# jgslunde/Lanczos

Measured on AMD Instinct MI355X. Metric: Lanczos iterations/sec + SpMV GB/s vs HBM roofline, n=1e7 5-pt Laplacian k=200, higher is better.
Workload: dtype f64

## Files before the change

### lanczos_amd/csrc/lz_api.hip

```cpp
#include <atomic>
#include <cstring>
#include <deque>
#include <unordered_map>

#include "lz_context.h"

using namespace lz;

namespace lz {
namespace api {

std::string g_create_error;


RcclApi g_rccl;

std::string g_rccl_path;
const char* load_rccl() {
  if (g_rccl.lib) return nullptr;
  void* lib = nullptr;
  std::vector<std::string> cand;
  if (const char* e = getenv("LZ_RCCL_PATH")) cand.push_back(e);
  Dl_info info;
  if (dladdr(reinterpret_cast<const void*>(static_cast<hipError_t (*)(void**, size_t)>(&hipMalloc)), &info) && info.dli_fname) {
    std::string dir(info.dli_fname);
    const size_t slash = dir.rfind('/');
    if (slash != std::string::npos) {
      dir.resize(slash);
      cand.push_back(dir + "/librccl.so.1");
      cand.push_back(dir + "/librccl.so");
    }
  }
  cand.push_back("/opt/rocm/lib/librccl.so.1");
  for (const auto& c : cand) {
    lib = dlopen(c.c_str(), RTLD_NOW | RTLD_LOCAL);
    if (lib) {
      g_rccl_path = c;
      break;
    }
  }
  if (!lib) return "cannot dlopen librccl next to the HIP runtime in use (set LZ_RCCL_PATH)";
#define LZ_SYM(field, name)                                          \
  g_rccl.field = reinterpret_cast<decltype(g_rccl.field)>(dlsym(lib, name)); \
  if (!g_rccl.field) return "missing RCCL symbol " name;
  LZ_SYM(GetUniqueId, "ncclGetUniqueId")
  LZ_SYM(CommInitRank, "ncclCommInitRank")
  LZ_SYM(CommDestroy, "ncclCommDestroy")
  LZ_SYM(AllReduce, "ncclAllReduce")
  LZ_SYM(AllGather, "ncclAllGather")
  LZ_SYM(Send, "ncclSend")
  LZ_SYM(Recv, "ncclRecv")
  LZ_SYM(GroupStart, "ncclGroupStart")
  LZ_SYM(GroupEnd, "ncclGroupEnd")
  LZ_SYM(GetErrorString, "ncclGetErrorString")
#undef LZ_SYM
  g_rccl.lib = lib;
  return nullptr;
}

int fail(lz_handle h, int code, const std::string& msg) {
  if (h)
    h->err = msg;
  else
    g_create_error = msg;
  return code;
}

int64_t skew_stride(lz_handle h, int64_t ld) {
  if (h->tune[12] == 1) return ld;
  return ((ld / kPadDoubles) & 1) ? ld : ld + kPadDoubles;
}

int check_launch(lz_handle h, const char* what) {
  hipError_t e = hipGetLastError();
  if (e != hipSuccess) return fail(h, LZ_ERR_HIP, std::string(what) + ": " + hipGetErrorString(e));
  if (h->tap_what && std::strcmp(what, h->tap_what) == 0)
    LZ_HIP(h, hipMemcpyAsync(h->d_tap, h->d_part, h->tap_count * sizeof(double), hipMemcpyDeviceToDevice, h->stream));
  return LZ_OK;
}

int upload(lz_handle h, void* dst, const void* src, size_t bytes) {
  LZ_HIP(h, hipMemcpyAsync(dst, src, bytes, hipMemcpyHostToDevice, h->stream));
  return LZ_OK;
}
int upload2d(lz_handle h, void* dst, size_t dpitch, const void* src, size_t spitch, size_t width, size_t height) {
  LZ_HIP(h, hipMemcpy2DAsync(dst, dpitch, src, spitch, width, height, hipMemcpyHostToDevice, h->stream));
  return LZ_OK;
}

namespace {
struct RoctxApi {
  int (*push)(const char*) = nullptr;
  int (*pop)() = nullptr;
  bool tried = false;
};
RoctxApi g_roctx;
const char* const kClassNames[LZ_K_COUNT] = {"lz:spmv", "lz:qtw", "lz:update", "lz:three_term", "lz:final", "lz:comm", "lz:ritz"};
bool roctx_on() {
  if (!g_roctx.tried) {
    g_roctx.tried = true;
    const char* e = getenv("LZ_ROCTX");
    if (e && e[0] == '1') {
      void* lib = dlopen("librocprofiler-sdk-roctx.so", RTLD_NOW | RTLD_GLOBAL);
      if (!lib) lib = dlopen("libroctx64.so", RTLD_NOW | RTLD_GLOBAL);
      if (lib) {
        g_roctx.push = reinterpret_cast<int (*)(const char*)>(dlsym(lib, "roctxRangePushA"));
        g_roctx.pop = reinterpret_cast<int (*)()>(dlsym(lib, "roctxRangePop"));
      }
    }
  }
  return g_roctx.push && g_roctx.pop;
}
}

Scope::Scope(lz_handle h_, int cls_, double bytes, double flops) : h(h_), cls(cls_) {
  if (roctx_on()) {
    g_roctx.push(kClassNames[cls]);
    marked = true;
  }
  h->acc.bytes[cls] += bytes;
  h->acc.flops[cls] += flops;
  h->acc.launches[cls] += 1;
  on = (h->flags & LZ_FLAG_PROFILE) != 0 && h->prof_iter;
  if (on) {
    h->acc.timed_bytes[cls] += bytes;
    h->acc.timed_launches[cls] += 1;
    if (!h->free_events.empty()) {
      a = h->free_events.back().first;
      b = h->free_events.back().second;
      h->free_events.pop_back();
    } else {
      if (hipEventCreate(&a) != hipSuccess || hipEventCreate(&b) != hipSuccess) {
        on = false;
        return;
      }
    }
    hipEventRecord(a, h->stream);
  }
}
Scope::~Scope() {
  if (marked) g_roctx.pop();
  if (on) {
    hipEventRecord(b, h->stream);
    h->events.push_back({cls, a, b});
  }
}

namespace {
struct BigBuf {
  size_t bytes = 0;
  std::vector<hipMemGenericAllocationHandle_t> chunks;
  std::vector<size_t> sizes;
};
std::mutex g_big_mu;
std::unordered_map<void*, BigBuf> g_big;
std::atomic<bool> g_vmm_off{false};
constexpr size_t kBigChunk = (size_t)2 << 30;
constexpr size_t kBigAlign = (size_t)2 << 20;

struct Quarantined {
  void* va;
  size_t bytes;
};
std::deque<Quarantined> g_quarantine;
size_t g_quarantine_bytes = 0;
constexpr size_t kQuarantineBytes = (size_t)16 << 40;

void big_release(void* va, BigBuf& b) {
  size_t off = 0;
  for (size_t k = 0; k < b.chunks.size(); ++k) {
    (void)hipMemUnmap(static_cast<char*>(va) + off, b.sizes[k]);
    (void)hipMemRelease(b.chunks[k]);
    off += b.sizes[k];
  }
  (void)hipMemAddressFree(va, b.bytes);
  static const bool reuse_ok = getenv("LZ_VMM_ADDRESS_REUSE") != nullptr;
  if (reuse_ok) return;
  void* q = nullptr;
  if (hipMemAddressReserve(&q, b.bytes, kBigAlign, va, 0) == hipSuccess && q) {
    if (q != va) {
      (void)hipMemAddressFree(q, b.bytes);
      if (getenv("LZ_DEBUG_VMM")) fprintf(stderr, "[vmm] quarantine of %p (%zu bytes) not honoured: got %p\n", va, b.bytes, q);
      return;
    }
    std::vector<Quarantined> old;
    {
      std::lock_guard<std::mutex> lk(g_big_mu);
      g_quarantine.push_back({q, b.bytes});
      g_quarantine_bytes += b.bytes;
      while (g_quarantine_bytes > kQuarantineBytes && g_quarantine.size() > 1) {
        old.push_back(g_quarantine.front());
        g_quarantine_bytes -= g_quarantine.front().bytes;
        g_quarantine.pop_front();
      }
    }
    for (const Quarantined& o : old) (void)hipMemAddressFree(o.va, o.bytes);
  } else {
    (void)hipGetLastError();
    if (getenv("LZ_DEBUG_VMM")) fprintf(stderr, "[vmm] quarantine of %p (%zu bytes): reservation failed\n", va, b.bytes);
  }
}
}

hipError_t big_alloc(int dev, void** out, size_t bytes) {
  *out = nullptr;
  static const bool no_vmm = getenv("LZ_NO_VMM") != nullptr;
  if (!no_vmm && !g_vmm_off.load() && bytes >= kBigMinBytes) {
    const size_t total = (bytes + kBigAlign - 1) / kBigAlign * kBigAlign;
    hipMemAllocationProp prop;
    memset(&prop, 0, sizeof prop);
    prop.type = hipMemAllocationTypePinned;
    prop.location.type = hipMemLocationTypeDevice;
    prop.location.id = dev;
    hipMemAccessDesc acc;
    acc.location.type = hipMemLocationTypeDevice;
    acc.location.id = dev;
    acc.flags = hipMemAccessFlagsProtReadWrite;
    void* va = nullptr;
    if (hipMemAddressReserve(&va, total, kBigAlign, nullptr, 0) == hipSuccess && va) {
      BigBuf b;
      b.bytes = total;
      bool ok = true, oom = false;
      for (size_t off = 0; off < total && ok; off += kBigChunk) {
        const size_t sz = std::min(kBigChunk, total - off);
        hipMemGenericAllocationHandle_t hh;
        hipError_t e = hipMemCreate(&hh, sz, &prop, 0);
        if (e != hipSuccess) {
          ok = false;
          oom = e == hipErrorOutOfMemory;
          break;
        }
        b.chunks.push_back(hh);
        b.sizes.push_back(sz);
        if (hipMemMap(static_cast<char*>(va) + off, sz, 0, hh, 0) != hipSuccess) {
          (void)hipMemRelease(hh);
          b.chunks.pop_back();
          b.sizes.pop_back();
          ok = false;
          break;
        }
        if (hipMemSetAccess(static_cast<char*>(va) + off, sz, &acc, 1) != hipSuccess) ok = false;
      }
      if (ok) {
        std::lock_guard<std::mutex> lk(g_big_mu);
        g_big.emplace(va, std::move(b));
        *out = va;
        return hipSuccess;
      }
      big_release(va, b);
      (void)hipGetLastError();
      if (oom) return hipErrorOutOfMemory;
    } else {
      (void)hipGetLastError();
    }
  }
  return hipMalloc(out, bytes);
}

void big_vmm_disable() { g_vmm_off.store(true); }

hipError_t big_free(void* p) {
  if (!p) return hipSuccess;
  BigBuf b;
  {
    std::lock_guard<std::mutex> lk(g_big_mu);
    auto it = g_big.find(p);
    if (it == g_big.end()) return hipFree(p);
    b = std::move(it->second);
    g_big.erase(it);
  }
  hipError_t e = hipDeviceSynchronize();
  big_release(p, b);
  return e;
}

int drain_events(lz_handle h) {
  if (h->events.empty() && !h->run_timed) return LZ_OK;
  LZ_HIP(h, hipStreamSynchronize(h->stream));
  for (auto& e : h->events) {
    float ms = 0.f;
    LZ_HIP(h, hipEventElapsedTime(&ms, e.a, e.b));
    h->acc.ms[e.cls] += ms;
    h->free_events.push_back({e.a, e.b});
  }
  h->events.clear();
  if (h->run_timed) {
    float ms = 0.f;
    LZ_HIP(h, hipEventElapsedTime(&ms, h->run_a, h->run_b));
    h->acc.total_ms += ms;
    h->run_timed = false;
  }
  return LZ_OK;
}

int comm_allreduce(lz_handle h, double* dbuf, int64_t count) {
  if ((h->world <= 1 && !(h->tune[6] && h->comm_kind)) || count <= 0) return LZ_OK;
  Scope sc(h, LZ_K_COMM, 8.0 * count, 0);
  h->n_allreduce += 1;
  if (h->comm_kind == 1) {
    LZ_NCCL(h, g_rccl.AllReduce(dbuf, dbuf, (size_t)count, ncclDouble, ncclSum, h->comm, h->stream));
    return LZ_OK;
  }
  if (h->comm_kind == 2) {
    h->hbuf_a.resize((size_t)count);
    LZ_HIP(h, hipMemcpyAsync(h->hbuf_a.data(), dbuf, count * sizeof(double), hipMemcpyDeviceToHost, h->stream));
    LZ_HIP(h, hipStreamSynchronize(h->stream));
    h->host_syncs += 2;
    if (h->h_ar(h->h_user, h->hbuf_a.data(), count) != 0) return fail(h, LZ_ERR_COMM, "host all-reduce callback failed");
    LZ_HIP(h, hipMemcpyAsync(dbuf, h->hbuf_a.data(), count * sizeof(double), hipMemcpyHostToDevice, h->stream));
    LZ_HIP(h, hipStreamSynchronize(h->stream));
    return LZ_OK;
  }
  return fail(h, LZ_ERR_STATE, "world > 1 but no communicator initialised");
}

int comm_exchange_x(lz_handle h, int j, const double** x_out) {
  double* vj = h->d_V + (int64_t)j * h->ldv;
  *x_out = vj;
  if (h->world <= 1 && !(h->tune[6] && h->comm_kind)) return LZ_OK;
  if (h->xmode == 1) {
    if (h->peers.empty()) return LZ_OK;
    Scope sc(h, LZ_K_COMM, 8.0 * (h->total_send + h->total_recv), 0);
    h->n_exchange += 1;
    const bool direct = h->all_contig && h->comm_kind == 1;
    if (!direct) {
      launch_gather(vj, h->d_send_idx, h->total_send, h->d_sendbuf, h->stream);
      LZ_TRY(check_launch(h, "gather"));
    }
    double* ghost = vj + h->rows_pad;
    if (h->comm_kind == 1) {
      LZ_NCCL(h, g_rccl.GroupStart());
      for (size_t p = 0; p < h->peers.size(); ++p) {
        const double* src = direct ? vj + h->sstart[p] : h->d_sendbuf + h->soff[p];
        if (h->scount[p] > 0)
          LZ_NCCL(h, g_rccl.Send(src, (size_t)h->scount[p], ncclDouble, h->peers[p], h->comm, h->stream));
        if (h->rcount[p] > 0)
          LZ_NCCL(h, g_rccl.Recv(ghost + h->roff[p], (size_t)h->rcount[p], ncclDouble, h->peers[p], h->comm, h->stream));
      }
      LZ_NCCL(h, g_rccl.GroupEnd());
    } else {
      h->hbuf_a.resize((size_t)std::max<int64_t>(h->total_send, 1));
      h->hbuf_b.resize((size_t)std::max<int64_t>(h->total_recv, 1));
      LZ_HIP(h, hipMemcpyAsync(h->hbuf_a.data(), h->d_sendbuf, h->total_send * sizeof(double), hipMemcpyDeviceToHost, h->stream));
      LZ_HIP(h, hipStreamSynchronize(h->stream));
      h->host_syncs += 2;
      if (h->h_ex(h->h_user, (int)h->peers.size(), h->peers.data(), h->hbuf_a.data(), h->scount.data(), h->hbuf_b.data(),
                  h->rcount.data()) != 0)
        return fail(h, LZ_ERR_COMM, "host halo-exchange callback failed");
      LZ_HIP(h, hipMemcpyAsync(ghost, h->hbuf_b.data(), h->total_recv * sizeof(double), hipMemcpyHostToDevice, h->stream));
      LZ_HIP(h, hipStreamSynchronize(h->stream));
    }
    return LZ_OK;
  }
  if (h->xmode == 2) {
    Scope sc(h, LZ_K_COMM, 8.0 * h->ag_chunk * h->world, 0);
    h->n_exchange += 1;
    if (h->comm_kind == 1) {
      LZ_NCCL(h, g_rccl.AllGather(vj, h->d_xfull, (size_t)h->ag_chunk, ncclDouble, h->comm, h->stream));
    } else {
      h->hbuf_a.resize((size_t)h->ag_chunk);
      h->hbuf_b.resize((size_t)(h->ag_chunk * h->world));
      LZ_HIP(h, hipMemcpyAsync(h->hbuf_a.data(), vj, h->ag_chunk * sizeof(double), hipMemcpyDeviceToHost, h->stream));
      LZ_HIP(h, hipStreamSynchronize(h->stream));
      h->host_syncs += 2;
      if (h->h_ag(h->h_user, h->hbuf_a.data(), h->hbuf_b.data(), h->ag_chunk) != 0)
        return fail(h, LZ_ERR_COMM, "host all-gather callback failed");
      LZ_HIP(h, hipMemcpyAsync(h->d_xfull, h->hbuf_b.data(), h->ag_chunk * h->world * sizeof(double), hipMemcpyHostToDevice, h->stream));
      LZ_HIP(h, hipStreamSynchronize(h->stream));
    }
    *x_out = h->d_xfull;
    return LZ_OK;
  }
  return fail(h, LZ_ERR_STATE, "world > 1 but neither lz_set_halo nor lz_set_allgather was called");
}

int require_basis(lz_handle h, int j) {
  if (!h->d_V) return fail(h, LZ_ERR_STATE, "no basis allocated (call lz_run or lz_basis_alloc first)");
  if (j < 0 || j >= h->n) return fail(h, LZ_ERR_ARG, "basis row index out of range");
  return LZ_OK;
}

}
}

using namespace lz::api;

extern "C" {

int lz_version(void) { return 100; }

int lz_device_count(int* count) {
  if (!count) return LZ_ERR_ARG;
  int c = 0;
  hipError_t e = hipGetDeviceCount(&c);
  if (e != hipSuccess) {
    *count = 0;
    g_create_error = std::string("hipGetDeviceCount: ") + hipGetErrorString(e);
    return LZ_ERR_NODEVICE;
  }
  *count = c;
  return LZ_OK;
}

int lz_create(lz_handle* out, int device_id) {
  if (!out) return fail(nullptr, LZ_ERR_ARG, "out is NULL");
  *out = nullptr;
  int c = 0;
  hipError_t e = hipGetDeviceCount(&c);
  if (e != hipSuccess || c <= 0)
    return fail(nullptr, LZ_ERR_NODEVICE,
                std::string("no HIP device available: ") + (e != hipSuccess ? hipGetErrorString(e) : "device count is 0"));
  if (device_id < 0 || device_id >= c) return fail(nullptr, LZ_ERR_ARG, "device_id out of range");
  e = hipSetDevice(device_id);
  if (e != hipSuccess) return fail(nullptr, LZ_ERR_HIP, std::string("hipSetDevice: ") + hipGetErrorString(e));
  lz_context* h = new lz_context();
  h->dev = device_id;
  memset(&h->acc, 0, sizeof(h->acc));
  hipDeviceProp_t prop;
  if (hipGetDeviceProperties(&prop, device_id) == hipSuccess) h->name = std::string(prop.name) + " (" + prop.gcnArchName + ")";
  e = hipStreamCreateWithFlags(&h->stream, hipStreamNonBlocking);
  if (e != hipSuccess) {
    delete h;
    return fail(nullptr, LZ_ERR_HIP, std::string("hipStreamCreate: ") + hipGetErrorString(e));
  }
  hipEventCreate(&h->run_a);
  hipEventCreate(&h->run_b);
  *out = h;
  return LZ_OK;
}

int lz_destroy(lz_handle h) {
  if (!h) return LZ_OK;
  hipSetDevice(h->dev);
  hipStreamSynchronize(h->stream);
  if (h->comm && g_rccl.CommDestroy) g_rccl.CommDestroy(h->comm);
  big_free(h->csr.rowptr);
  big_free(h->csr.colidx);
  big_free(h->csr.vals);
  big_free(h->csr.rowblk);
  pb_free(h->csr.pb);
  pb_free(h->csrT.pb);
  ell_free(h->csr);
  ell_free(h->csrT);
  big_free(h->d_dense);
  big_free(h->d_V);
  big_free(h->d_r);
  big_free(h->d_r2);
  big_free(h->d_alpha);
  big_free(h->d_beta);
  big_free(h->d_c);
  big_free(h->d_nrm2);
  big_free(h->d_part);
  big_free(h->csrT.rowptr);
  big_free(h->csrT.colidx);
  big_free(h->csrT.vals);
  big_free(h->csrT.rowblk);
  big_free(h->d_B3);
  big_free(h->d_s);
  big_free(h->d_gamma);
  big_free(h->d_bi);
  big_free(h->d_xtmp);
  big_free(h->d_Y);
  big_free(h->d_S);
  big_free(h->d_rclk);
  big_free(h->d_gram);
  big_free(h->d_gclk);
  big_free(h->d_send_idx);
  big_free(h->d_sendbuf);
  big_free(h->d_xfull);
  big_free(h->d_om);
  big_free(h->d_os);
  big_free(h->d_osi);
  big_free(h->d_tap);
  big_free(h->d_omi);
  big_free(h->res_V);
  big_free(h->res_Y);
  orth_free(h->trl);
  big_free(h->d_tW);
  orth_free(h->trl_wk);
  gk_free(h);
  z_free(h);
  expm_free(h);
  minres_free(h);
  lsmr_free(h);
  bicgstab_free(h);
  gmres_free(h);
  big_free(h->poly.d_rot);
  big_free(h->poly.d_acc);
  big_free(h->poly.d_coef);
  if (h->h_pinned) hipHostFree(h->h_pinned);
  xfer_free(h->xfer);
  if (h->cstream) {
    hipStreamSynchronize(h->cstream);
    hipStreamDestroy(h->cstream);
    hipEventDestroy(h->e_bnd);
    hipEventDestroy(h->e_halo);
  }
  for (auto& e : h->events) {
    hipEventDestroy(e.a);
    hipEventDestroy(e.b);
  }
  for (auto& e : h->free_events) {
    hipEventDestroy(e.first);
    hipEventDestroy(e.second);
  }
  if (h->run_a) hipEventDestroy(h->run_a);
  if (h->run_b) hipEventDestroy(h->run_b);
  hipStreamDestroy(h->stream);
  delete h;
  return LZ_OK;
}

const char* lz_last_error(lz_handle h) { return h ? h->err.c_str() : g_create_error.c_str(); }

int lz_set_options(lz_handle h, int flags) {
  if (!h) return LZ_ERR_ARG;
#ifndef LZ_KBENCH
  if (flags & LZ_FLAG_QTW_MFMA)
    return fail(h, LZ_ERR_ARG, "lz_set_options: LZ_FLAG_QTW_MFMA (the 16x16x4 Q^T w arm, 20 % slower) was retired from the product library (build with KBENCH=1)");
#endif
  h->flags = flags;
  return LZ_OK;
}

int lz_set_tuning(lz_handle h, int index, int value) {
  if (!h) return LZ_ERR_ARG;
  if (index < 0 || index >= 24) return fail(h, LZ_ERR_ARG, "lz_set_tuning: knob index out of range");
  if ((index == 1 && value >= 20) || (index == 3 && value != 0) || (index == 9 && value >= 10))
    return fail(h, LZ_ERR_ARG, "lz_set_tuning: the timing-only ablation arms were removed in round 5 (their measurements are in profiles/)");
#ifndef LZ_KBENCH
  if ((index == 15 && value >= 2 && (value < 6 || value > 11)) || (index == 9 && value >= 2) || (index == 11 && value >= 2) || (index == 22 && value >= 2))
    return fail(h, LZ_ERR_ARG, "lz_set_tuning: this A/B arm was retired from the product library (build with KBENCH=1)");
#endif
  if (value < 0) return fail(h, LZ_ERR_ARG, "lz_set_tuning: negative value");
  h->tune[index] = value;
  return LZ_OK;
}

int lz_runtime_info(char* buf, size_t buflen) {
  if (!buf || buflen == 0) return LZ_ERR_ARG;
  Dl_info info;
  const char* hip = "";
  if (dladdr(reinterpret_cast<const void*>(static_cast<hipError_t (*)(void**, size_t)>(&hipMalloc)), &info) && info.dli_fname) hip = info.dli_fname;
  snprintf(buf, buflen, "hip=%s;rccl=%s", hip, g_rccl_path.c_str());
  return LZ_OK;
}

int lz_device_synchronize(lz_handle h) {
  if (!h) return LZ_ERR_ARG;
  LZ_HIP(h, hipSetDevice(h->dev));
  LZ_HIP(h, hipDeviceSynchronize());
  return LZ_OK;
}

int lz_device_memory(lz_handle h, int64_t* free_bytes, int64_t* total_bytes) {
  if (!h || !free_bytes || !total_bytes) return LZ_ERR_ARG;
  LZ_HIP(h, hipSetDevice(h->dev));
  size_t f = 0, t = 0;
  LZ_HIP(h, hipMemGetInfo(&f, &t));
  *free_bytes = (int64_t)f;
  *total_bytes = (int64_t)t;
  return LZ_OK;
}

int lz_device_name(lz_handle h, char* buf, size_t buflen) {
  if (!h || !buf || buflen == 0) return LZ_ERR_ARG;
  snprintf(buf, buflen, "%s", h->name.c_str());
  return LZ_OK;
}

int64_t lz_padded_rows(int64_t rows) { return round_up(rows, kPadDoubles); }

int lz_comm_load(void) {
  const char* e = load_rccl();
  if (e) return fail(nullptr, LZ_ERR_COMM, e);
  return LZ_OK;
}

int lz_comm_unique_id(void* id, size_t id_bytes) {
  if (!id || id_bytes < sizeof(ncclUniqueId)) return fail(nullptr, LZ_ERR_ARG, "id buffer must hold at least 128 bytes");
  const char* e = load_rccl();
  if (e) return fail(nullptr, LZ_ERR_COMM, e);
  ncclUniqueId uid;
  ncclResult_t r = g_rccl.GetUniqueId(&uid);
  if (r != ncclSuccess) return fail(nullptr, LZ_ERR_COMM, std::string("ncclGetUniqueId: ") + g_rccl.GetErrorString(r));
  memset(id, 0, id_bytes);
  memcpy(id, &uid, sizeof(uid));
  return LZ_OK;
}

int lz_comm_init_rccl(lz_handle h, int world, int rank, const void* id, size_t id_bytes) {
  if (!h) return LZ_ERR_ARG;
  if (world < 1 || rank < 0 || rank >= world || !id || id_bytes < sizeof(ncclUniqueId))
    return fail(h, LZ_ERR_ARG, "bad world/rank/id");
  const char* e = load_rccl();
  if (e) return fail(h, LZ_ERR_COMM, e);
  LZ_HIP(h, hipSetDevice(h->dev));
  ncclUniqueId uid;
  memcpy(&uid, id, sizeof(uid));
  LZ_NCCL(h, g_rccl.CommInitRank(&h->comm, world, uid, rank));
  if (world > 1) big_vmm_disable();
  h->world = world;
  h->rank = rank;
  h->comm_kind = 1;
  return LZ_OK;
}

int lz_comm_init_host(lz_handle h, int world, int rank, lz_host_allreduce_fn ar, lz_host_exchange_fn ex,
                      lz_host_allgather_fn ag, void* user) {
  if (!h) return LZ_ERR_ARG;
  if (world < 1 || rank < 0 || rank >= world || !ar) return fail(h, LZ_ERR_ARG, "bad world/rank/callbacks");
  h->world = world;
  h->rank = rank;
  h->comm_kind = 2;
  h->h_ar = ar;
  h->h_ex = ex;
  h->h_ag = ag;
  h->h_user = user;
  return LZ_OK;
}

}
int lz::api::basis_alloc(lz_handle h, int n, int zero_rows) {
  if (!h) return LZ_ERR_ARG;
  if (h->kind == 0) return fail(h, LZ_ERR_STATE, "no matrix set (lz_set_csr / lz_set_dense)");
  if (n < 1) return fail(h, LZ_ERR_ARG, "n must be >= 1");
  if (h->world > 1 && h->xmode == 0) return fail(h, LZ_ERR_STATE, "multi-rank run needs lz_set_halo or lz_set_allgather");
  LZ_HIP(h, hipSetDevice(h->dev));
  LZ_HIP(h, hipStreamSynchronize(h->stream));
  const size_t vsz = (size_t)n * (size_t)h->ldv;
  const bool fresh = !h->d_V || h->n != n;
  if (fresh) {
    double* adopted = nullptr;
    {
      std::lock_guard<std::mutex> lk(h->res_mu);
      if (h->res_V && h->res_V_count >= vsz) {
        adopted = h->res_V;
        h->res_V = nullptr;
        h->res_V_count = 0;
      }
    }
    if (adopted) {
      LZ_TRY(dev_free(h, h->d_V));
      h->d_V = adopted;
    } else {
      LZ_TRY(dev_alloc(h, h->d_V, vsz));
    }
    if (getenv("LZ_DEBUG_PTR")) fprintf(stderr, "[lz] basis %p (%zu bytes, ld %lld)\n", (void*)h->d_V, vsz * sizeof(double), (long long)h->ldv);
    LZ_TRY(dev_alloc(h, h->d_r, (size_t)h->ldv));
    LZ_TRY(dev_alloc(h, h->d_r2, (size_t)h->ldv));
    LZ_TRY(dev_alloc(h, h->d_alpha, (size_t)n + 1));
    LZ_TRY(dev_alloc(h, h->d_beta, (size_t)n + 1));
    LZ_TRY(dev_alloc(h, h->d_c, 2 * ((size_t)2 * qtw_ldp(n + 2) + 8)));
    LZ_TRY(dev_alloc(h, h->d_nrm2, 2));
  }
  if (fresh) {
    if (h->tune[13] == 1) LZ_HIP(h, hipMemsetAsync(h->d_V, 0xFF, vsz * sizeof(double), h->stream));
    if (h->ldv > h->rows_pad)
      LZ_HIP(h, hipMemset2DAsync(h->d_V + h->rows_pad, (size_t)h->ldv * sizeof(double), 0, (size_t)(h->ldv - h->rows_pad) * sizeof(double),
                                 (size_t)n, h->stream));
  }
  h->n = n;
  h->os_step_n = 0;
  h->qplan = plan_qtw(h->rows_pad, h->flags, h->tune, n);
  size_t need = (size_t)(n + 16) * (size_t)h->qplan.P;
  if (h->flags & LZ_FLAG_ONE_REDUCE) need = (size_t)2 * qtw_ldp(n + 2) * (size_t)h->qplan.P;
  if ((h->flags & LZ_FLAG_ONE_REDUCE) && (h->flags & LZ_FLAG_REORTH_PARTIAL)) need = onered_part_off(h) + std::max<size_t>(need, 8192);
  if (h->qplan.G <= 8) need = std::max<size_t>(need, fused_coff(h) + (size_t)(n + 16) * (size_t)h->qplan.G);
  need = std::max<size_t>(need, 8192);
  need = std::max<size_t>(need, (size_t)(h->rows / 4 + 64));
  need = std::max<size_t>(need, (size_t)h->csr.n_rowblk + 64);
  if (h->csr.pb) need = std::max<size_t>(need, (size_t)pb_num_partials(h->csr.pb) + 64);
  if (h->csrT.pb) need = std::max<size_t>(need, (size_t)pb_num_partials(h->csrT.pb) + 64);
  LZ_TRY(ensure_part(h, need));
  LZ_HIP(h, hipMemsetAsync(h->d_V, 0, (size_t)std::min(zero_rows, n) * (size_t)h->ldv * sizeof(double), h->stream));
  LZ_HIP(h, hipMemsetAsync(h->d_r, 0, (size_t)h->ldv * sizeof(double), h->stream));
  LZ_HIP(h, hipMemsetAsync(h->d_r2, 0, (size_t)h->ldv * sizeof(double), h->stream));
  LZ_HIP(h, hipMemsetAsync(h->d_alpha, 0, ((size_t)n + 1) * sizeof(double), h->stream));
  LZ_HIP(h, hipMemsetAsync(h->d_beta, 0, ((size_t)n + 1) * sizeof(double), h->stream));
  LZ_HIP(h, hipMemsetAsync(h->d_c, 0, 2 * ((size_t)2 * qtw_ldp(n + 2) + 8) * sizeof(double), h->stream));
  LZ_HIP(h, hipMemsetAsync(h->d_nrm2, 0, 2 * sizeof(double), h->stream));
  LZ_HIP(h, hipStreamSynchronize(h->stream));
  return LZ_OK;
}
// ... 195 lines not shown
```

### lanczos_amd/csrc/lz_context.h

```cpp
#pragma once

#include <dlfcn.h>
#include <rccl/rccl.h>

#include <algorithm>
#include <chrono>
#include <cmath>
#include <cstdio>
#include <cstdlib>
#include <cstring>
#include <functional>
#include <mutex>
#include <system_error>
#include <thread>

#include "lz_internal.h"

using lz::CsrDev;
using lz::QtwPlan;
using lz::Xfer;

struct EventRec {
  int cls;
  hipEvent_t a, b;
};

struct RcclApi {
  void* lib = nullptr;
  ncclResult_t (*GetUniqueId)(ncclUniqueId*) = nullptr;
  ncclResult_t (*CommInitRank)(ncclComm_t*, int, ncclUniqueId, int) = nullptr;
  ncclResult_t (*CommDestroy)(ncclComm_t) = nullptr;
  ncclResult_t (*AllReduce)(const void*, void*, size_t, ncclDataType_t, ncclRedOp_t, ncclComm_t, hipStream_t) = nullptr;
  ncclResult_t (*AllGather)(const void*, void*, size_t, ncclDataType_t, ncclComm_t, hipStream_t) = nullptr;
  ncclResult_t (*Send)(const void*, size_t, ncclDataType_t, int, ncclComm_t, hipStream_t) = nullptr;
  ncclResult_t (*Recv)(void*, size_t, ncclDataType_t, int, ncclComm_t, hipStream_t) = nullptr;
  ncclResult_t (*GroupStart)() = nullptr;
  ncclResult_t (*GroupEnd)() = nullptr;
  const char* (*GetErrorString)(ncclResult_t) = nullptr;
};

struct TrlPoly {
  enum Kind { kNone, kFilter, kSeries } kind = kNone;
  int degree = 0, coef_cap = 0;
  double c = 0.0, inv_e = 0.0;
  double* d_coef = nullptr;
  double* d_rot = nullptr;
  double* d_acc = nullptr;
  int64_t ld = 0;
  void clear() { kind = kNone, degree = 0; }
};

struct OrthBasis {
  double* B = nullptr;
  double* w = nullptr;
  int64_t len = 0, pad = 0, ld = 0;
  int nrows = 0;
  int planes = 1;
};
struct OrthWork {
  double* sm = nullptr;
  int* gate = nullptr;
  double* part = nullptr;
  size_t part_cap = 0;
};
struct OrthSmallHead {
  int64_t c1, c2, nrm2, end;
};
inline OrthSmallHead orth_small_head(int nrows, int planes = 1) {
  const int64_t cl = lz::qtw_ldp(planes * (nrows + 1)) + 16;
  return {0, cl, 2 * cl, 2 * cl + 8};
}

struct GkState {
  bool set = false;
  CsrDev A, AT;
  lz::DenseDev D;
  int m = 0;
  int u_ready = -1;
  OrthBasis U;
  OrthBasis V;
  OrthWork wk;
};

struct ZState {
  int kind = 0;
  int64_t n = 0, nnz = 0;
  int32_t* rowptr = nullptr;
  int32_t* colidx = nullptr;
  double* vals = nullptr;
  int group = 1;
  double* xtmp = nullptr;
  int64_t xtmp_pad = 0;
  OrthBasis B;
  OrthWork wk;
  int m = 0;
};

struct ExpmState {
  OrthBasis B;
  OrthWork wk;
  int m = 0;
  int form = 0;
  int product = 0;
  double* xtmp = nullptr;
  int64_t xtmp_pad = 0;
};

struct MinresState {
  double* vec = nullptr;
  double* ds = nullptr;
  int* di = nullptr;
  double* part = nullptr;
  size_t part_cap = 0;
  double* hist = nullptr;
  int hist_cap = 0;
  int64_t ld = 0;
  bool live = false;
  int steps = 0;
  int done = 0;
};

struct LsmrState {
  double* bvec = nullptr;
  double* xvec = nullptr;
  double* ds = nullptr;
  int* di = nullptr;
  double* part = nullptr;
  double* hist = nullptr;
  int hist_cap = 0;
  int64_t blen = 0, bpad = 0, xlen = 0, xpad = 0;
  int transposed = 0;
  bool live = false;
  bool pending = false;
  int steps = 0;
  int done = 0;
};

struct BicgstabState {
  double* vec = nullptr;
  double* ds = nullptr;
  int* di = nullptr;
  double* part = nullptr;
  size_t part_cap = 0;
  double* hist = nullptr;
  int hist_cap = 0;
  int64_t ld = 0;
  bool live = false;
  bool fresh = false;
  int steps = 0;
  int done = 0;
};

struct GmresState {
  OrthBasis B;
  OrthWork wk;
  int m = 0;
  double* vec = nullptr;
  int* di = nullptr;
  double* rpart = nullptr;
  double* hist = nullptr;
  int hist_cap = 0;
  double* chist = nullptr;
  int chist_cap = 0;
  bool live = false;
  bool fresh = false;
  bool pending = false;
  int hcol = 0;
  int iters = 0, cycles = 0, done = 0;
};

struct lz_context {
  int dev = 0;
  hipStream_t stream = nullptr;
  std::string err;
  std::string name;
  int flags = 0;
  int tune[24] = {0};

  int64_t Mg = 0, row0 = 0, rows = 0, ncols_ext = 0;
  int64_t rows_pad = 0;
  int64_t ldv = 0;

  int kind = 0;
  CsrDev csr;
  double* d_dense = nullptr;
  int64_t dense_lda = 0;

  int n = 0;
  double* d_V = nullptr;
  double* d_r = nullptr;
  double* d_r2 = nullptr;
  double* d_alpha = nullptr;
  double* d_beta = nullptr;
  double* d_c = nullptr;
  double* d_nrm2 = nullptr;
  double* d_part = nullptr;
  size_t part_cap = 0;
  double* d_xtmp = nullptr;
  QtwPlan qplan;

  CsrDev csrT;
  bool has_T = false;
  bool T_declared = false;
  double* d_B3 = nullptr;
  int bi_n = 0;
  double* d_s = nullptr;
  double* d_gamma = nullptr;
  double* d_bi = nullptr;

  double* d_Y = nullptr;
  int64_t y_rows = 0;
  int y_n = 0;
  double* d_S = nullptr;
  int s_npad = 0;
  uint64_t* d_rclk = nullptr;
  double* d_gram = nullptr;
  size_t gram_cap = 0;
  uint64_t* d_gclk = nullptr;
  bool gram_sym_last = false;
  bool y_chunked = false;
  int64_t y_chunk = 0;
  int64_t y_cap = 0;

  int world = 1, rank = 0;
  int comm_kind = 0;
  ncclComm_t comm = nullptr;
  lz_host_allreduce_fn h_ar = nullptr;
  lz_host_exchange_fn h_ex = nullptr;
  lz_host_allgather_fn h_ag = nullptr;
  void* h_user = nullptr;
  std::vector<double> hbuf_a, hbuf_b;
  int xmode = 0;
  std::vector<int32_t> peers;
  std::vector<int64_t> scount, rcount, soff, roff;
  std::vector<int64_t> sstart;
  bool all_contig = false;
  hipStream_t cstream = nullptr;
  hipEvent_t e_bnd = nullptr, e_halo = nullptr;
  int halo_inflight_j = -1;
  std::vector<std::pair<int64_t, int64_t>> bnd_ranges, int_ranges;
  int64_t total_send = 0, total_recv = 0;
  int64_t n_allreduce = 0, n_exchange = 0;
  int64_t n_allreduce_last = 0, n_exchange_last = 0;
  int32_t* d_send_idx = nullptr;
  double* d_sendbuf = nullptr;
  int64_t ag_chunk = 0;
  double* d_xfull = nullptr;

  std::vector<EventRec> events;
  std::vector<std::pair<hipEvent_t, hipEvent_t>> free_events;
  hipEvent_t run_a = nullptr, run_b = nullptr;
  bool run_timed = false;
  int last_sweeps = 0;
  std::vector<int> sweep_log;
  int last_misses = 0;
  int last_engine = 0;
  int r_state = 0;
  Xfer* xfer = nullptr;
  double* h_pinned = nullptr;
  double* d_os = nullptr;
  int* d_osi = nullptr;
  int os_n = 0;
  int os_step_n = 0;
  const char* tap_what = nullptr;
  double* d_tap = nullptr;
  size_t tap_cap = 0, tap_count = 0;
  int last_gate_trips = 0;
  int last_os_fused = 0;
  int last_os_pairs = 0;
  int last_pair_abandoned = 0;
  bool pair_tripped = false;
  int last_os_quads = 0;
  int last_quad_abandoned = 0;
  bool quad_tripped = false;
  double* d_om = nullptr;
  int* d_omi = nullptr;
  int om_n = 0;
  int om_run_n = 0;
  int64_t host_syncs = 0;
  std::mutex res_mu;
  double* res_V = nullptr;
  size_t res_V_count = 0;
  double* res_Y = nullptr;
  size_t res_Y_count = 0;
  OrthBasis trl;
  int trl_m = 0;
  int trl_b = 1;
  double* d_tW = nullptr;
  OrthWork trl_wk;
  TrlPoly poly;
  GkState gk;
  ZState z;
  ExpmState ex;
  MinresState mr;
  LsmrState ls;
  BicgstabState bc;
  GmresState gm;
  bool prof_iter = true;
  lz_timings acc;
};

namespace lz {
namespace api {

extern std::string g_create_error;
extern RcclApi g_rccl;
extern std::string g_rccl_path;
const char* load_rccl();

int fail(lz_handle h, int code, const std::string& msg);

#define LZ_HIP(h, call)                                                                                   \
  do {                                                                                                    \
    hipError_t e_ = (call);                                                                               \
    if (e_ != hipSuccess)                                                                                 \
      return fail(h, e_ == hipErrorOutOfMemory ? LZ_ERR_NOMEM : LZ_ERR_HIP,                               \
                  std::string(#call) + ": " + hipGetErrorString(e_));                                     \
  } while (0)

#define LZ_NCCL(h, call)                                                                                  \
  do {                                                                                                    \
    ncclResult_t r_ = (call);                                                                             \
    if (r_ != ncclSuccess) return fail(h, LZ_ERR_COMM, std::string(#call) + ": " + g_rccl.GetErrorString(r_)); \
  } while (0)

#define LZ_TRY(expr)          \
  do {                        \
    int rc_ = (expr);         \
    if (rc_ != LZ_OK) return rc_; \
  } while (0)

int64_t skew_stride(lz_handle h, int64_t ld);
int check_launch(lz_handle h, const char* what);

constexpr size_t kBigMinBytes = (size_t)256 << 20;
hipError_t big_alloc(int dev, void** out, size_t bytes);
hipError_t big_free(void* p);
void big_vmm_disable();

template <class T>
inline int dev_free(lz_handle h, T*& p) {
  if (p) {
    LZ_HIP(h, big_free(p));
    p = nullptr;
  }
  return LZ_OK;
}

template <class T>
inline int dev_alloc(lz_handle h, T*& p, size_t count) {
  LZ_TRY(dev_free(h, p));
  void* q = nullptr;
  LZ_HIP(h, big_alloc(h->dev, &q, std::max<size_t>(count, 1) * sizeof(T)));
  p = static_cast<T*>(q);
  return LZ_OK;
}

int upload(lz_handle h, void* dst, const void* src, size_t bytes);
int upload2d(lz_handle h, void* dst, size_t dpitch, const void* src, size_t spitch, size_t width, size_t height);

struct Scope {
  lz_handle h;
  int cls;
  hipEvent_t a = nullptr, b = nullptr;
  bool on;
  bool marked = false;
  Scope(lz_handle h_, int cls_, double bytes, double flops);
  ~Scope();
};
int drain_events(lz_handle h);

int comm_allreduce(lz_handle h, double* dbuf, int64_t count);
int comm_exchange_x(lz_handle h, int j, const double** x_out);

int ensure_part(lz_handle h, size_t need);
double spmv_bytes(lz_handle h, bool ell = false);
double spmv_flops(lz_handle h);
int step_spmv(lz_handle h, int j, double* alpha_dst = nullptr, bool reduce = true, int* np_out = nullptr);
int step_reorth(lz_handle h, int j, int nrows, bool scale, int beta_idx, bool in_run_loop = false);
int step_three_term(lz_handle h, int j, int jm1, const double* d_alpha, const double* d_beta, bool need_norm = true, int* np_out = nullptr,
                    double* r = nullptr, const char* what = "three_term");
size_t fused_coff(lz_handle h);
size_t onered_part_off(lz_handle h);
int breakdown_status(lz_handle h, int n, const double* alpha_out, const double* beta_out);

int basis_alloc(lz_handle h, int n, int zero_rows);
int require_basis(lz_handle h, int j);
inline size_t y_doubles(int64_t rows, int n) { return (size_t)(round_up(rows, 16) + 16) * (size_t)n + 64; }

int fill_csr_meta(lz_handle h, CsrDev& A, const int32_t* rowptr_host, int64_t rows_local, int64_t ncols_ext, int64_t nnz, int fixed_k,
                  int max_nnz);
int upload_csr(lz_handle h, CsrDev& A, const char* who, int64_t rows, int64_t ncols, int64_t nnz, const int32_t* rowptr,
               const int32_t* colidx, const double* vals, int* fixed_k_out, int* max_nnz_out);

void gk_free(lz_handle h);
hipError_t gk_product(lz_handle h, int transpose, const double* x, double* y, int64_t pad);

int z_drop_matrix(lz_handle h);
void z_free(lz_handle h);
void z_matvec(lz_handle h, const double* x, double* y, int64_t ld);

void expm_free(lz_handle h);

void minres_free(lz_handle h);

void lsmr_free(lz_handle h);

void bicgstab_free(lz_handle h);

void gmres_free(lz_handle h);

QtwPlan orth_plan(lz_handle h, const OrthBasis& b);
int orth_dots(lz_handle h, const OrthBasis& b, const OrthWork& wk, const QtwPlan& plan, int n, double* c, const int* gate = nullptr);
int orth_store(lz_handle h, const OrthBasis& b, const OrthWork& wk, const QtwPlan& plan, int k, const char* what);
enum class OrthPass2 {
  kGated,
  kForced,
  kUngated,
};
int orth_cgs_step(lz_handle h, const OrthBasis& b, const OrthWork& wk, const QtwPlan& plan, int nb, double* proj, double* norm_slot,
                  OrthPass2 pass2);
int orth_upload_x(lz_handle h, const OrthBasis& b, const double* x);
int orth_get_vectors(lz_handle h, const OrthBasis& b, int k, double* out);
int orth_set_rows(lz_handle h, const OrthBasis& b, const char* who, const char* top, int j0, int count, const double* rows, int64_t ld);
int orth_get_rows(lz_handle h, const OrthBasis& b, const char* who, const char* top, int j0, int count, double* rows, int64_t ld);
void to_planar(const double* z, int64_t n, double* re, double* im);
void to_interleaved(const double* re, const double* im, int64_t n, double* z);
int orth_resid_norms(lz_handle h, const OrthBasis& b, const OrthWork& wk, int k, const double* theta, double* out,
                     const std::function<hipError_t(int)>& product);
size_t orth_part_need(const OrthBasis& b, const QtwPlan& plan, int m);
int orth_part_reserve(lz_handle h, OrthWork& wk, size_t need);
void orth_free(OrthBasis& b);
void orth_free(OrthWork& wk);

}
}
```

### lanczos_amd/csrc/lz_internal.h

```cpp
#pragma once

#include <hip/hip_runtime.h>
#include <stdint.h>

#include <algorithm>
#include <string>
#include <system_error>
#include <thread>
#include <vector>

#include "lanczos_hip.h"

namespace lz {

constexpr int kWave = 64;
constexpr int kTPB = 256;
constexpr int kPadDoubles = 32;
constexpr int kNumCU = 256;
constexpr int kNumXCD = 8;

inline int64_t round_up(int64_t x, int64_t m) { return (x + m - 1) / m * m; }

int xfer_threads();
template <class F>
// ... 68 lines not shown
  double* S = nullptr;
  int64_t R = 0, C = 0, ld = 0;
  bool stored_t = false;
  int rd_form = 0, rd_group = 0, rd_nseg = 0;
  int64_t rd_seg = 0;
  int cs_form = 0, cs_group = 0, cs_nslab = 0;
  int64_t cs_slab = 0;
  double* rd_part = nullptr;
  double* cs_part = nullptr;
};
constexpr int kDenseTileCols = 128;
constexpr int kDenseShortMax = 128;
constexpr int kDenseShortRows = 4;
constexpr int kDenseMediumMax = 1024;
constexpr int kDenseSegRows = 4;
constexpr int kDenseSegMaxRows = 768;
constexpr int kDenseFoldSub = 16;
void dense_plan(DenseDev& D, int force_rd, int force_cs, int seg_knob, int slab_knob);
hipError_t launch_dense_rowdot(const DenseDev& D, const double* x, double* out, int64_t pad, hipStream_t s);
hipError_t launch_dense_colsum(const DenseDev& D, const double* u, double* out, int64_t pad, hipStream_t s);

hipError_t pb_build(const CsrDev& A, const int32_t* rowptr_host, PbDev** out, hipStream_t s, int cap_knob = 0, int groups = 0);
void pb_free(PbDev*& pb);
int pb_num_partials(const PbDev* pb);
void pb_layout_info(const PbDev* pb, int64_t* np, int* in_bytes_x2, int* diag);
int launch_spmv_pb(const CsrDev& A, const PbDev* pb, const double* x, double* y, const double* x_own, double* part, hipStream_t s);

int launch_spmv_csr(const CsrDev& A, const double* x, double* y, const double* x_own, double* part, int flags,
                    hipStream_t s);
hipError_t ell_build(CsrDev& A, int variant, hipStream_t s, int coding = 0, bool plain_fallback = true);
void ell_free(CsrDev& A);
bool ell_usable(const CsrDev& A, int flags);
struct EllCode {
  const double* diag = nullptr;
  const uint8_t* cls = nullptr;
  const int32_t* off = nullptr;
  const double* val = nullptr;
  int ncls = 0;
};
struct SpmvScale {
  const double* r = nullptr;
  const double* nrm2 = nullptr;
  double* vj = nullptr;
  double* beta_slot = nullptr;
  const int* gate = nullptr;
};
struct SpmvCheb {
  const double* xprev = nullptr;
  double* z = nullptr;
  const double* coef = nullptr;
  int i = 0, degree = 0;
  double c = 0.0;
  const double* acc_in = nullptr;
  double* acc = nullptr;
  double inv_e = 0.0;
};
int launch_spmv_ell(const CsrDev& A, const double* x, double* y, const double* x_own, double* part, hipStream_t s,
                    const SpmvScale* sc = nullptr, const SpmvCheb* ch = nullptr);
struct StencilArgs {
  int Nx, Ny, Nz, negate, pot_kind, renumber, nranges;
  int64_t row0, rows_local;
  double tf, w[4], par[8];
  int64_t gstart[16], glen[16], gext[16];
};
void launch_build_stencil3d(const StencilArgs& a, int points, const double* pot, int32_t* rowptr, int32_t* colidx, double* vals,
                            hipStream_t s);
int launch_gemv_dense(const double* A, int64_t M, int64_t cols, int64_t lda, const double* x, const double* x_own, double* y,
                      double* part, hipStream_t s);

void launch_final_sum(const double* part, int n, double* out, hipStream_t s);
inline int qtw_ldp(int nrows) { return (nrows + 15) & ~15; }
void launch_final_rows(const double* part, int nrows, int G, double* c, hipStream_t s, bool transposed = false, const int* gate = nullptr);
void launch_final_rows_t(const double* part, int G, int ldp, int nout, double* c, hipStream_t s, const int* gate = nullptr);
struct FinalMulti {
  const double* part[4];
  int n[4];
  double* out[4];
};
void launch_final_sum_multi(const FinalMulti& fm, int count, hipStream_t s);

struct QtwPlan {
  int64_t L = 0;
  int G = 0;
  int P = 0;
  bool mfma = false;
  int family = 2;
  int variant = 0;
};
QtwPlan plan_qtw(int64_t len, int flags, const int* tune, int nrows_max);
struct QtwFuse {
  const double* apart = nullptr;
  int np = 0;
  int jprev = 0, jprev2 = -1;
  const double* beta_prev = nullptr;
  double* alpha_out = nullptr;
  double* r_out = nullptr;
  const int* gate = nullptr;
  unsigned* ticket = nullptr;
  double* c_out = nullptr;
};
hipError_t launch_qtw(double* V, int64_t ldv, int64_t len, int nrows, int j, const double* r, const double* nrm2,
                      double* beta_slot, const QtwPlan& plan, double* part, int mode, hipStream_t s, const QtwFuse* fuse = nullptr);
void launch_update(double* V, int64_t ldv, int64_t len, int nrows, int j, const double* c, const double* r_fused,
                   double* beta, int variant, hipStream_t s, int64_t pos_lo = 0, int64_t pos_hi = -1, int raw_c = 0,
                   int64_t pos_lo_b = 0, int64_t pos_hi_b = 0,
                   int cG = 0, int cldp = 0, const int* gate = nullptr,
                   const double* usub = nullptr, const double* asub = nullptr);
void launch_scale_store(double* vj, const double* r, const double* nrm2, double* beta_slot, int64_t len, hipStream_t s, const int* gate = nullptr);

constexpr double kOneSweepTau = 1e-14;
constexpr int kOneSweepMaxN = 1536;
constexpr int kOneSweepFusedMaxN = kOneSweepMaxN - 16;
__host__ __device__ inline double os_predict_one(int i, int j, int n, const double* H, const double* G, double a, double bj, double bn) {
  double s;
  if (i < j) {
    s = 0.0;
    for (int l = 0; l <= i + 1; ++l) s += H[(int64_t)i * n + l] * G[(int64_t)j * n + l];
  } else {
    s = a;
  }
  s = s - a * G[(int64_t)j * n + i];
  if (j > 0) s = s - bj * G[(int64_t)(j - 1) * n + i];
  return s / bn;
}
__host__ __device__ inline double os_post_one(int i, int j, int n, const double* G, const double* d, const double* chat, double cs) {
  double s = (2.0 - cs) * d[i];
  for (int l = 0; l < j; ++l) s -= chat[l] * G[(int64_t)l * n + i];
  return s;
}
int os_sweep_blocks(int64_t len);
int launch_os_sweep(int mode, double* V, int64_t ldv, int64_t len, int j, const double* coef, const double* r, const double* nrm2,
                    double* beta_slot, double* part, const int* gate, hipStream_t s, double* dst = nullptr, const double* alpha_prev = nullptr,
                    const double* beta_prev = nullptr);
void launch_os_post(const double* d, const double* chat, double* G, double* H, int n, int j, double* nrm2, double tau, double* g, int* ist,
                    double* elog, bool fused, hipStream_t s);
void launch_os_sum_predict(const double* part, int np, double* sum_out, const double* G, double* H, int n, int j, const double* alpha_j,
                           const double* beta_j, double* chat, bool fused, bool predict, hipStream_t s);
constexpr int kOneSweepPairMaxLdp = 1024;
int os_pair_ldp(int j);
int os_pair_sweep_blocks(int64_t len, bool wide16);
void launch_os_pair_predict(const double* part, int np, double* alpha_out, const double* nrm2, const double* chat, const double* G, double* H,
                            int n, int j, double* kap, double* p, hipStream_t s);
int launch_os_pair_sweep(double* V, int64_t ldv, int64_t len, int j, const double* chat, const double* kap, const double* w, double* y,
                         const double* nrm2, const double* alpha0, double* part, bool wide16, hipStream_t s);
void launch_os_pair_post(const double* d, int ldp, const double* chat, const double* kap, const double* p, double* G, double* H, int n, int j,
                         double* nrm2, const double* alpha_j, double tau, int* ist, double* elog, hipStream_t s);
constexpr int kOneSweepQuadLds = 65536;
inline size_t os_quad_lds_bytes(int ldp) { return (size_t)(kTPB / 64) * 4 * ldp * sizeof(double); }
inline int os_quad_max_ldp() { return (int)(kOneSweepQuadLds / os_quad_lds_bytes(1)); }
int os_quad_ldp(int j);
int os_quad_sweep_blocks(int64_t len, bool wide8);
void launch_os_quad_predict(const double* part, int np, double* nrm2, const double* chat, const double* G, const double* H, int n, int j,
                            const double* alpha, const double* beta, double* gout, int ldg, hipStream_t s);
int launch_os_quad_sweep(double* V, int64_t ldv, int64_t len, int j, const double* g, int ldg, const double* z, const double* nrm2, double* part,
                         bool wide8, hipStream_t s);
hipError_t launch_os_quad_post(const double* d, int ldp, const double* g, int ldg, double* G, double* H, int n, int j, const double* nrm2,
                               const double* alpha, double* beta, double tau, int* ist, double* elog, hipStream_t s);
inline size_t omega_state_doubles(int n) { return (size_t)2 + (n + 2) + 3 * (size_t)(n + 1); }
inline size_t omega_state_ints(int n) { return (size_t)2 + n + 1; }
void launch_omega(const double* part, int np, double* nrm2, const double* alpha, int jn, int n, double* st, int* ist, hipStream_t s,
                  double* c_clear = nullptr);
inline size_t omega_onered_ints(int n) { return (size_t)4 + n + 2; }
void launch_partial_onered_post(double* buf, double* bufn, int nzero_next, int m, int ldp, double* alpha_slot, double* nrm2, const double* alpha,
                                int j, int n, double* st, int* ist, double kappa, double* beta_prev, double* uu_keep, hipStream_t s);
int launch_three_term_self(double* r, const double* u, const double* vm, const double* beta, int64_t len, double* part, hipStream_t s);
void launch_fused_prepare(double* c, int j, double* beta_slot, hipStream_t s);
void launch_onereduce_prepare(double* buf, int m, int ldp, double* alpha_slot, double* bad, double* beta_prev, double* uu_keep, hipStream_t s);
void launch_onereduce_finish(const double* buf, int ldp, double* alpha_last, double* beta_last, const double* uu_keep, hipStream_t s);
int launch_three_term(double* r, const double* vj, const double* vjm1, const double* alpha, const double* beta,
                      int64_t len, double* part, hipStream_t s);
void launch_gather(const double* x, const int32_t* idx, int64_t n, double* buf, hipStream_t s);

void launch_bi(int first, int pend, int dots, double* x, double* y, const double* xs, const double* ys, const double* f,
               const double* ap, const double* bp, const double* Sp, const double* a, const double* b, int64_t len, double* part,
               int epi, double* S, double* fo, double* o0, double* o1, unsigned* ticket, hipStream_t s, const double* pend_part = nullptr,
               bool defer_fold = false);
void launch_bi_two_term(int sub, int dots, double* r, double* sv, const double* u, const double* v, const double* c0, const double* c1,
                        const double* da, const double* db, int64_t len, double* part, double* fo, double* o0, double* o1,
                        unsigned* ticket, hipStream_t s);
struct Xfer;
void xfer_free(Xfer*& x);
hipError_t xfer_d2h(int dev, hipStream_t stream, Xfer*& state, void* dst, size_t dpitch, const void* src, size_t spitch, size_t width,
                    size_t height);
int xfer_threads();

void launch_bi_mem_safe(double* xrow, const double* B, int64_t ldv, int n, int j, int64_t len, double* coef, hipStream_t s);
int bi_partials_needed();

hipError_t launch_ritz_gemm(const double* V, int64_t ldv, int64_t rows, int n, const double* Spad, int npad, double* Y,
                            int64_t ldy, hipStream_t s, int variant = 0, unsigned long long* clk = nullptr);
void launch_ritz_gemm_cols(const double* V, int64_t ldv, int64_t rows, int kcount, const double* B, int ldb, int ncols, double* Y,
                           int64_t ldy, hipStream_t s);
int launch_gram(const double* Y, int64_t ldy, int64_t rows, int n, double* part, int nz_max, hipStream_t s);
void launch_sum_slices(const double* part, int nz, int64_t count, double* out, hipStream_t s);
constexpr int kGramMaxSlices = 768;
size_t gram_scratch_doubles(int n);
bool launch_gram_sym(const double* Y, int64_t ldy, int64_t rows, int n, double* part, double* out, hipStream_t s,
                     unsigned long long* clk = nullptr, int nz_override = 0,
                     int variant = 0);
int launch_ritz_quality(const CsrDev& A, const double* Y, int64_t ldy, int n, double* part, hipStream_t s);
void launch_extract_column(const double* Y, int64_t ldy, int col, int64_t rows, int64_t rows_pad, double* x, hipStream_t s);

hipError_t launch_trl_restart(double* V, int64_t ldv, int64_t rows, int m, int kk, const double* S, hipStream_t s);
int launch_trl_cgs(const double* V, int64_t ldv, int64_t len, int nrows, const double* c, double* r, double* part, const int* gate, hipStream_t s);
int trl_cgs_blocks(int64_t len);
void launch_trl_post(int mode, const double* part, int np, const double* c, int j, double* nrm2, double* proj, int* gate, int force, hipStream_t s);
inline int trl_band_run(int r0, int b) { return (r0 * b + 15) & ~15; }
int trl_band_dots_blocks(int64_t len, int b);
hipError_t launch_trl_band_dots(const double* V, int64_t ldv, int64_t len, int r0, const double* W, int64_t ldw, int b, double* part, hipStream_t s);
int trl_band_update_blocks(int64_t len);
int launch_trl_band_update(const double* V, int64_t ldv, int64_t len, int r0, const double* C, double* W, int64_t ldw, int b, double* part,
                           hipStream_t s);
void launch_trl_band_proj(const double* C1, const double* C2, int r0, int b, int nb, double* proj, int ldf, hipStream_t s);
int launch_trl_resid_csr(const CsrDev& A, const double* Y, int64_t ldy, int k, const double* theta, double* part, hipStream_t s);
int launch_trl_resid_diff(const double* y, const double* x, int64_t rows, const double* theta, int i, double* part, hipStream_t s);
int launch_trl_resid_cplx_csr(const CsrDev& A, const double* Y, int64_t ldy, int k, const double* re, const double* im, double* part,
                              hipStream_t s);
int launch_trl_resid_cplx_diff(const double* yr, const double* yi, const double* xr, const double* xi, int64_t rows, const double* re,
                               const double* im, int i, double* part, hipStream_t s);
void launch_trl_rownorm(const double* part, int G, int k, double* out, hipStream_t s);
void launch_cheb_step(double* wz, const double* y, const double* x, const double* coef, int i, int degree, double c, int64_t rows,
                      int64_t len, hipStream_t s);
void launch_cheb_series_step(double* wz, const double* y, const double* x, const double* acc_in, double* acc_out, const double* mu, int i,
                             int last, double inv_e, double c, int64_t rows, int64_t len, hipStream_t s);

void launch_zspmv_csr(const int32_t* rowptr, const int32_t* colidx, const double* vals, int64_t rows, int group, const double* xr,
                      const double* xi, double* yr, double* yi, hipStream_t s);
void launch_zgemv(const double* A, int64_t n, const double* xr, const double* xi, double* yr, double* yi, hipStream_t s);
constexpr int kZMaxRows = 65;
int zdots_blocks(int64_t len);
int launch_zdots(const double* V, int64_t ldv, int64_t len, int nb, const double* w, double* part, const int* gate, hipStream_t s);
int zcgs_blocks(int64_t len);
int launch_zcgs(const double* V, int64_t ldv, int64_t len, int nb, const double* c, double* w, double* part, const int* gate, hipStream_t s);
int launch_zresid_diff(const double* y, const double* x, int64_t ld, int64_t n, const double* theta, int i, double* part, hipStream_t s);

struct SmallArgs {
  int kind;
  const int32_t* rowptr;
  const int32_t* colidx;
  const double* vals;
  const int32_t* rowblk;
  int nparts;
  const double* dense;
  int64_t lda;
  int rows, rows_pad, n;
  int64_t ldv;
  double* V;
  const double* x0;
  double* y;
  double* drow;
  double* pc;
  double* alpha;
  double* beta;
  unsigned* bar;
  unsigned* xcc;
  unsigned long long zero;
};

constexpr int kSmallMaxPadRows = 1280;
int small_grid(int rows_pad);
hipError_t launch_small_run(const SmallArgs& a, int nb, bool local, hipStream_t s);
hipError_t launch_small_step(const SmallArgs& a, int mode, int j, int nb, hipStream_t s);

}
```

### lanczos_amd/csrc/lz_loops.hip

```cpp
#include "lz_context.h"

using namespace lz;
using namespace lz::api;

namespace lz {
namespace api {

inline double* basis_row(lz_handle h, int j) { return h->d_V + (int64_t)j * h->ldv; }
inline int beta_index(int n, int j) { return (j + n - 2) % (n - 1); }
inline double* beta_slot(lz_handle h, int n, int j) { return h->d_beta + beta_index(n, j); }
inline bool iter_sampled(lz_handle h, int j) {
  const int pstride = h->tune[7] > 1 ? h->tune[7] : 1;
  return (j % pstride) == pstride / 2;
}
inline void begin_iter(lz_handle h, int j) { h->prof_iter = iter_sampled(h, j); }

int ensure_part(lz_handle h, size_t need) {
  if (need <= h->part_cap) return LZ_OK;
  LZ_TRY(dev_alloc(h, h->d_part, need));
  h->part_cap = need;
  return LZ_OK;
}

double spmv_bytes(lz_handle h, bool ell) {
// ... 218 lines not shown
    LZ_TRY(check_launch(h, "onereduce_finish"));
  }
  return LZ_OK;
}

size_t onered_part_off(lz_handle h) {
  size_t np = std::max<size_t>((size_t)h->rows / 4 + 2, (size_t)std::max(h->csr.n_rowblk, 1));
  if (h->csr.pb) np = std::max<size_t>(np, (size_t)pb_num_partials(h->csr.pb));
  return (np + 64 + 63) / 64 * 64;
}

size_t fused_coff(lz_handle h) {
  const size_t npmax = std::max<size_t>((size_t)h->rows / 4 + 2, (size_t)std::max(h->csr.n_rowblk, 1)) + 64;
  return (npmax + 63) / 64 * 64;
}

int run_loop_fused_small(lz_handle h, int n) {
  const double M = (double)h->rows;
  const size_t coff = fused_coff(h);
  int np = 0;
  LZ_TRY(step_spmv(h, 0, nullptr, false, &np));
  for (int j = 0; j < n; ++j) {
    begin_iter(h, j);
    const QtwFuse fz = qtw_prologue_fuse(h, j, h->d_part, np);
    h->qplan.variant = 0;
    {
      Scope sc(h, LZ_K_QTW, 8.0 * j * M + 40.0 * M, 2.0 * (j + 1) * M + 4.0 * M);
      LZ_HIP(h, launch_qtw(h->d_V, h->ldv, h->rows_pad, j + 1, j, h->d_r, nullptr, nullptr, h->qplan, h->d_part + coff, 4, h->stream, &fz));
      LZ_TRY(check_launch(h, "qtw(fused three-term)"));
    }
    {
      Scope sc(h, LZ_K_UPDATE, 8.0 * j * M + 16.0 * M, 2.0 * (j + 1) * M);
      launch_update(h->d_V, h->ldv, h->rows_pad, j + 1, j, h->d_part + coff, h->d_r2, beta_slot(h, n, j), 0, h->stream, 0, -1, 2, 0, 0, h->qplan.G,
                    qtw_ldp(j + 1));
      LZ_TRY(check_launch(h, "update(fused reduction)"));
    }
    LZ_TRY(step_spmv(h, j, nullptr, false, &np));
  }
  LZ_TRY(step_final_sum(h, np, h->d_alpha + (n - 1), "final_sum(alpha)"));
  h->r_state = 2;
  return LZ_OK;
}


constexpr int64_t kThreeTermFusedMaxRows = 4'000'000;
int run_loop_three_term_fused(lz_handle h, int n) {
  const double M = (double)h->rows;
  LZ_TRY(step_spmv(h, 0));
  for (int j = 0; j < n; ++j) {
    begin_iter(h, j);
    const QtwFuse fz = qtw_prologue_fuse(h, j, nullptr, 0);
    h->qplan.variant = 0;
    {
      Scope sc(h, LZ_K_QTW, 8.0 * j * M + 40.0 * M, 2.0 * (j + 1) * M + 4.0 * M);
      LZ_HIP(h, launch_qtw(h->d_V, h->ldv, h->rows_pad, j + 1, j, h->d_r, nullptr, nullptr, h->qplan, h->d_part, 4, h->stream, &fz));
      LZ_TRY(check_launch(h, "qtw(three-term in the prologue)"));
    }
    {
      Scope sc(h, LZ_K_FINAL, 0, 0);
      launch_final_rows(h->d_part, j + 1, h->qplan.P, h->d_c, h->stream, h->qplan.family == 2);
      LZ_TRY(check_launch(h, "final_rows"));
    }
    LZ_TRY(comm_allreduce(h, h->d_c, j + 1));
    {
      Scope sc(h, LZ_K_UPDATE, 8.0 * j * M + 16.0 * M, 2.0 * (j + 1) * M);
      launch_update(h->d_V, h->ldv, h->rows_pad, j + 1, j, h->d_c, h->d_r2, beta_slot(h, n, j), 0, h->stream, 0, -1, 1);
      LZ_TRY(check_launch(h, "update"));
    }
    LZ_TRY(step_spmv(h, j));
  }
  h->r_state = 2;
  return LZ_OK;
}

#ifdef LZ_KBENCH
constexpr int kSmallStepMaxN = 64;
bool small_args(lz_handle h, int n, SmallArgs& sa) {
  memset(&sa, 0, sizeof sa);
  sa.kind = h->kind;
  if (h->kind == 2) {
    sa.dense = h->d_dense;
    sa.lda = h->dense_lda;
    sa.nparts = (int)((h->rows + 3) / 4);
  } else {
    const CsrDev& A = h->csr;
    const bool fixed = !(h->flags & LZ_FLAG_SPMV_STREAM) && (A.fixed_k == 5 || A.fixed_k == 7);
    const bool ell_other_grouping = A.ell_default && !(A.ell_coded && fixed);
    if (A.pb || ell_other_grouping || A.max_row_nnz > 32 || (fixed && A.fixed_rb != 512)) return false;
    sa.rowptr = A.rowptr;
    sa.colidx = A.colidx;
    sa.vals = A.vals;
    sa.rowblk = fixed ? nullptr : A.rowblk;
    sa.nparts = fixed ? (int)((h->rows + 511) / 512) : A.n_rowblk;
  }
  if (sa.nparts > 1024 || h->part_cap < (size_t)(2048 + h->rows_pad)) return false;
  sa.rows = (int)h->rows;
  sa.rows_pad = (int)h->rows_pad;
  sa.n = n;
  sa.ldv = h->ldv;
  sa.V = h->d_V;
  sa.y = h->d_r;
  sa.drow = h->d_part;
  sa.x0 = h->d_part + 2048;
  sa.pc = h->d_c;
  sa.alpha = h->d_alpha;
  sa.beta = h->d_beta;
  sa.bar = reinterpret_cast<unsigned*>(h->d_nrm2);
  sa.xcc = reinterpret_cast<unsigned*>(h->d_part + 3400);
  return true;
}
bool small_engine_applies(lz_handle h) {
  SmallArgs sa;
  return small_args(h, 2, sa);
}

int run_small_engine(lz_handle h, int n, const double* v0_local, bool steps, bool* ran) {
  SmallArgs sa;
  *ran = small_args(h, n, sa);
  if (!*ran) return LZ_OK;
  LZ_HIP(h, hipMemcpyAsync(h->d_part + 2048, h->d_V, (size_t)h->rows_pad * sizeof(double), hipMemcpyDeviceToDevice, h->stream));
  if (steps) {
    const int nb = h->kind == 2 ? (int)std::min<int64_t>(256, (h->rows + 3) / 4) : (int)std::max<int64_t>(1, (h->rows + kTPB - 1) / kTPB);
    const double Mr = (double)h->rows;
    LZ_HIP(h, launch_small_step(sa, 0, -1, nb, h->stream));
    for (int j = -1; j <= n - 2; ++j) {
      const int pstride = h->tune[7] > 1 ? h->tune[7] : 1;
      h->prof_iter = ((j + 1) % pstride) == pstride / 2;
      Scope sc(h, LZ_K_UPDATE, spmv_bytes(h) + 16.0 * (j + 2) * Mr + 40.0 * Mr, spmv_flops(h) + 4.0 * (j + 2) * Mr);
      LZ_HIP(h, launch_small_step(sa, 1, j, nb, h->stream));
    }
    h->prof_iter = true;
    LZ_HIP(h, launch_small_step(sa, 2, n - 1, 1, h->stream));
    return check_launch(h, "small_step");
  }
  h->acc.launches[LZ_K_FINAL] += 1;
  LZ_HIP(h, launch_small_run(sa, small_grid(sa.rows_pad), h->tune[15] == 2, h->stream));
  LZ_TRY(check_launch(h, "small_run"));
  unsigned status = 0;
  LZ_HIP(h, hipMemcpyAsync(&status, sa.bar + 2, sizeof status, hipMemcpyDeviceToHost, h->stream));
  LZ_HIP(h, hipStreamSynchronize(h->stream));
  if (status != 0) {
    if (getenv("LZ_DEBUG_TIMING")) fprintf(stderr, "[lz_run] small-problem engine gave up (status %u): multi-kernel path\n", status);
    *ran = false;
    LZ_TRY(basis_alloc(h, n, 1));
    LZ_HIP(h, hipMemcpyAsync(h->d_V, v0_local, (size_t)h->rows * sizeof(double), hipMemcpyHostToDevice, h->stream));
    LZ_HIP(h, hipEventRecord(h->run_a, h->stream));
  }
  return LZ_OK;
}
#endif

struct OneSweepState {
  double *G, *H, *chat, *g, *elog, *gq;
  int nb;
};
static void one_sweep_view(lz_handle h, int n, OneSweepState& st) {
  st.nb = os_sweep_blocks(h->rows_pad);
  st.G = h->d_os;
  st.H = st.G + (size_t)n * n;
  st.chat = st.H + (size_t)n * n;
  st.g = st.chat + n + 1;
  st.elog = st.g + 2 * n + 2;
  st.gq = st.elog + n + 1;
}
static int one_sweep_setup(lz_handle h, int n, OneSweepState& st, int pair_blocks = 0) {
  const size_t os_doubles = (size_t)2 * n * n + (size_t)5 * n + 8 + (size_t)4 * (n + 4);
  if (h->os_n < n) {
    LZ_TRY(dev_alloc(h, h->d_os, os_doubles));
    LZ_TRY(dev_alloc(h, h->d_osi, 8));
    h->os_n = n;
  }
  h->os_step_n = 0;
  one_sweep_view(h, n, st);
  LZ_TRY(ensure_part(h, (size_t)std::max(st.nb, 2 * pair_blocks) * qtw_ldp(n + 1) + 64));
  LZ_HIP(h, hipMemsetAsync(h->d_os, 0, os_doubles * sizeof(double), h->stream));
  LZ_HIP(h, hipMemsetAsync(h->d_osi, 0, 8 * sizeof(int), h->stream));
  return LZ_OK;
}
static int one_sweep_step(lz_handle h, int n, int j, const OneSweepState& st, bool fused) {
  const double M = (double)h->rows;
  double* dst = fused ? h->d_r2 : basis_row(h, j);
  {
    Scope sc(h, LZ_K_UPDATE, 8.0 * j * M + 16.0 * M, 4.0 * (j + 1) * M);
    if (fused)
      launch_os_sweep(2, h->d_V, h->ldv, h->rows_pad, j, st.chat, h->d_r, nullptr, nullptr, h->d_part, nullptr, h->stream, dst, h->d_alpha + (j - 1),
                      beta_slot(h, n, j - 1));
    else
      launch_os_sweep(0, h->d_V, h->ldv, h->rows_pad, j, st.chat, h->d_r, h->d_nrm2, beta_slot(h, n, j), h->d_part, nullptr, h->stream);
    LZ_TRY(check_launch(h, "one-sweep"));
  }
  {
    Scope sc(h, LZ_K_FINAL, 0, 0);
    const int nout = fused ? j + 2 : j + 1;
    launch_final_rows_t(h->d_part, st.nb, qtw_ldp(nout), nout, h->d_c, h->stream);
    LZ_TRY(check_launch(h, "final_rows(one-sweep)"));
    launch_os_post(h->d_c, st.chat, st.G, st.H, n, j, h->d_nrm2, kOneSweepTau, st.g, h->d_osi, st.elog, fused, h->stream);
    LZ_TRY(check_launch(h, "one-sweep post"));
  }
  {
    Scope sc(h, LZ_K_QTW, 0, 0);
    launch_os_sweep(1, h->d_V, h->ldv, h->rows_pad, j, fused ? st.g + n : st.g, nullptr, nullptr, nullptr, nullptr, h->d_osi, h->stream, dst);
    LZ_TRY(check_launch(h, "one-sweep correction"));
  }
  return LZ_OK;
}

int run_loop_one_sweep(lz_handle h, int n) {
  OneSweepState st;
  LZ_TRY(one_sweep_setup(h, n, st));
  LZ_TRY(warm_up(h, true));
  for (int j = 0; j < n; ++j) {
    begin_iter(h, j);
    LZ_TRY(one_sweep_step(h, n, j, st, false));
    LZ_TRY(step_spmv(h, j));
    int np = 0;
    LZ_TRY(step_three_term(h, j, j > 0 ? j - 1 : -1, h->d_alpha + j, beta_slot(h, n, j), false, &np));
    {
      Scope sc(h, LZ_K_FINAL, 0, 0);
      launch_os_sum_predict(h->d_part, np, h->d_nrm2, st.G, st.H, n, j, h->d_alpha + j, beta_slot(h, n, j), st.chat, false,
                            j + 1 < n, h->stream);
      LZ_TRY(check_launch(h, "final_sum(nrm2) + one-sweep predict"));
    }
  }
  h->r_state = 1;
  return LZ_OK;
}

bool one_sweep_fused_applies(lz_handle h, int n) {
  const bool one_rank = h->world == 1 && h->comm_kind == 0;
  return one_rank && h->kind == 1 && ell_usable(h->csr, h->flags) && (h->csr.fixed_k == 5 || h->csr.fixed_k == 7) && n <= kOneSweepFusedMaxN &&
         h->tune[15] != 7;
}
static int one_sweep_fused_iter(lz_handle h, int n, int j, const OneSweepState& st) {
  double* vj = basis_row(h, j);
  LZ_TRY(one_sweep_step(h, n, j, st, j > 0));
  int npa = 0;
  if (j == 0) {
    Scope sc(h, LZ_K_SPMV, spmv_bytes(h), spmv_flops(h));
    npa = launch_spmv_csr(h->csr, vj, h->d_r, vj, h->d_part, h->flags, h->stream);
    LZ_TRY(check_launch(h, "spmv"));
  } else {
    LZ_TRY(step_scaling_spmv(h, n, j, h->d_r2, h->d_r, h->d_osi + 2, &npa));
  }
  {
    Scope sc(h, LZ_K_FINAL, 0, 0);
    launch_os_sum_predict(h->d_part, npa, h->d_alpha + j, st.G, st.H, n, j, h->d_alpha + j, beta_slot(h, n, j), st.chat, true, j + 1 < n, h->stream);
    LZ_TRY(check_launch(h, "final_sum(alpha) + one-sweep predict"));
  }
  return LZ_OK;
}
static int one_sweep_fused_tail(lz_handle h, int n) {
  LZ_TRY(step_three_term(h, n - 1, n - 2, h->d_alpha + (n - 1), beta_slot(h, n, n - 1), true));
  h->r_state = 1;
  return LZ_OK;
}
int run_loop_one_sweep_fused(lz_handle h, int n) {
  OneSweepState st;
  LZ_TRY(one_sweep_setup(h, n, st));
  h->last_os_fused = 1;
  LZ_TRY(warm_up(h, true));
  for (int j = 0; j < n; ++j) {
    begin_iter(h, j);
    LZ_TRY(one_sweep_fused_iter(h, n, j, st));
  }
  return one_sweep_fused_tail(h, n);
}

bool one_sweep_pair_applies(lz_handle h, int n) {
  const int knob = h->tune[15];
  return one_sweep_fused_applies(h, n) && knob != 6 && n >= 4 && qtw_ldp(n + 1) <= kOneSweepPairMaxLdp && !h->pair_tripped;
}
static int one_sweep_pair_iter(lz_handle h, int n, int j, const OneSweepState& st, int nbp, bool wide16) {
  const double M = (double)h->rows;
  double* kap = st.g;
  double* pp = st.g + n + 1;
  const int* scale = h->d_osi + 2;
  h->prof_iter = iter_sampled(h, j) || iter_sampled(h, j + 1);
  LZ_TRY(step_three_term(h, j - 1, j - 2, h->d_alpha + (j - 1), h->d_beta + (j - 2), true));
  int npa = 0;
  LZ_TRY(step_scaling_spmv(h, n, j, h->d_r, h->d_r2, scale, &npa));
  const int ldp = os_pair_ldp(j);
  {
    Scope sc(h, LZ_K_FINAL, 0, 0);
    launch_os_pair_predict(h->d_part, npa, h->d_alpha + j, h->d_nrm2, st.chat, st.G, st.H, n, j, kap, pp, h->stream);
    LZ_TRY(check_launch(h, "one-sweep pair predict"));
  }
  {
    Scope sc(h, LZ_K_UPDATE, 8.0 * j * M + 40.0 * M, 8.0 * (j + 1) * M);
    launch_os_pair_sweep(h->d_V, h->ldv, h->rows_pad, j, st.chat, kap, h->d_r, h->d_r2, h->d_nrm2, h->d_alpha + j, h->d_part, wide16, h->stream);
    LZ_TRY(check_launch(h, "one-sweep pair walk"));
  }
  {
    Scope sc(h, LZ_K_FINAL, 0, 0);
    launch_final_rows_t(h->d_part, nbp, 2 * ldp, ldp + j + 2, h->d_c, h->stream);
    LZ_TRY(check_launch(h, "final_rows(one-sweep pair)"));
    launch_os_pair_post(h->d_c, ldp, st.chat, kap, pp, st.G, st.H, n, j, h->d_nrm2, h->d_alpha + j, kOneSweepTau, h->d_osi, st.elog, h->stream);
    LZ_TRY(check_launch(h, "one-sweep pair post"));
  }
  LZ_TRY(step_scaling_spmv(h, n, j + 1, h->d_r2, h->d_r, scale, &npa));
  {
    Scope sc(h, LZ_K_FINAL, 0, 0);
    launch_os_sum_predict(h->d_part, npa, h->d_alpha + (j + 1), st.G, st.H, n, j + 1, h->d_alpha + (j + 1), h->d_beta + j, st.chat, true,
                          j + 2 < n, h->stream);
    LZ_TRY(check_launch(h, "final_sum(alpha) + one-sweep predict"));
  }
  h->last_os_pairs += 1;
  return LZ_OK;
}
int run_loop_one_sweep_pair(lz_handle h, int n) {
  const bool wide16 = h->tune[15] == 9;
  OneSweepState st;
  const int nbp = os_pair_sweep_blocks(h->rows_pad, wide16);
  LZ_TRY(one_sweep_setup(h, n, st, nbp));
  h->last_os_fused = 1;
  LZ_TRY(warm_up(h, true));
  for (int j = 0; j < n;) {
    if (j < 2 || j + 1 >= n) {
      begin_iter(h, j);
      LZ_TRY(one_sweep_fused_iter(h, n, j, st));
      j += 1;
      continue;
    }
    LZ_TRY(one_sweep_pair_iter(h, n, j, st, nbp, wide16));
    j += 2;
  }
  return one_sweep_fused_tail(h, n);
}

bool one_sweep_quad_applies(lz_handle h, int n) {
  const int knob = h->tune[15];
  return one_sweep_pair_applies(h, n) && knob != 8 && knob != 9 && n >= 6 && os_quad_ldp(n - 4) <= os_quad_max_ldp() && !h->quad_tripped;
}
static int one_sweep_quad_iter(lz_handle h, int n, int j, const OneSweepState& st, int nbq, bool wide8) {
  const double M = (double)h->rows;
  const int ldg = n + 4;
  h->prof_iter = iter_sampled(h, j) || iter_sampled(h, j + 1) || iter_sampled(h, j + 2) || iter_sampled(h, j + 3);
  LZ_TRY(step_three_term(h, j - 1, j - 2, h->d_alpha + (j - 1), h->d_beta + (j - 2), true));
  double* src = h->d_r;
  double* dst = h->d_r2;
  int npz = 0;
  for (int t = 0; t < 3; ++t) {
    int npa = 0;
    LZ_TRY(step_scaling_spmv(h, n, j + t, src, dst, h->d_osi + 2, &npa));
    LZ_TRY(step_final_sum(h, npa, h->d_alpha + (j + t), "final_sum(alpha)"));
    LZ_TRY(step_three_term(h, j + t, j + t - 1, h->d_alpha + (j + t), h->d_beta + (j + t - 1), t < 2, &npz, dst));
    std::swap(src, dst);
  }
  const double* z = src;
  const int ldp = os_quad_ldp(j);
  {
    Scope sc(h, LZ_K_FINAL, 0, 0);
    launch_os_quad_predict(h->d_part, npz, h->d_nrm2, st.chat, st.G, st.H, n, j, h->d_alpha + j, h->d_beta + (j - 1), st.gq, ldg, h->stream);
    LZ_TRY(check_launch(h, "one-sweep group predict"));
  }
  {
    Scope sc(h, LZ_K_UPDATE, 8.0 * j * M + 64.0 * M, 16.0 * (j + 1) * M);
    launch_os_quad_sweep(h->d_V, h->ldv, h->rows_pad, j, st.gq, ldg, z, h->d_nrm2, h->d_part, wide8, h->stream);
    LZ_TRY(check_launch(h, "one-sweep group walk"));
  }
  {
    Scope sc(h, LZ_K_FINAL, 0, 0);
    launch_final_rows_t(h->d_part, nbq, 4 * ldp, 3 * ldp + j + 4, h->d_c, h->stream);
    LZ_TRY(check_launch(h, "final_rows(one-sweep group)"));
    LZ_HIP(h, launch_os_quad_post(h->d_c, ldp, st.gq, ldg, st.G, st.H, n, j, h->d_nrm2, h->d_alpha + j, h->d_beta + (j - 1), kOneSweepTau, h->d_osi,
                                  st.elog, h->stream));
    LZ_TRY(check_launch(h, "one-sweep group post"));
  }
  {
    double* vj = basis_row(h, j + 3);
    int npa = 0;
    {
      Scope sc(h, LZ_K_SPMV, spmv_bytes(h, true), spmv_flops(h));
      npa = launch_spmv_ell(h->csr, vj, h->d_r, vj, h->d_part, h->stream);
      LZ_TRY(check_launch(h, "spmv(ell)"));
    }
    Scope sc(h, LZ_K_FINAL, 0, 0);
    launch_os_sum_predict(h->d_part, npa, h->d_alpha + (j + 3), st.G, st.H, n, j + 3, h->d_alpha + (j + 3), h->d_beta + (j + 2), st.chat, true,
                          j + 4 < n, h->stream);
    LZ_TRY(check_launch(h, "final_sum(alpha) + one-sweep predict"));
  }
  h->last_os_quads += 1;
  return LZ_OK;
}
int run_loop_one_sweep_quad(lz_handle h, int n) {
  const bool wide8 = h->tune[15] == 11;
  OneSweepState st;
  const int nbp = os_pair_sweep_blocks(h->rows_pad, false), nbq = os_quad_sweep_blocks(h->rows_pad, wide8);
  LZ_TRY(one_sweep_setup(h, n, st, std::max(nbp, 2 * nbq)));
  h->last_os_fused = 1;
  LZ_TRY(warm_up(h, true));
  for (int j = 0; j < n;) {
    if (j >= 2 && n - j == 2 && (n - 2) % 4 == 2) {
      LZ_TRY(one_sweep_pair_iter(h, n, j, st, nbp, false));
      j += 2;
      continue;
    }
    if (j < 2 || j + 4 > n) {
      begin_iter(h, j);
      LZ_TRY(one_sweep_fused_iter(h, n, j, st));
      j += 1;
      continue;
    }
    LZ_TRY(one_sweep_quad_iter(h, n, j, st, nbq, wide8));
    j += 4;
  }
  return one_sweep_fused_tail(h, n);
}

static const char* one_sweep_step_refusal(lz_handle h, int n, int j, int form) {
  const bool full_fused = (h->flags & LZ_FLAG_FUSED_NORM) && !(h->flags & LZ_FLAG_REORTH_PARTIAL);
  if (h->tune[15] == 7) return "one-sweep step: tuning knob 15 is 7 (never the fused one-sweep form)";
  if (n > kOneSweepFusedMaxN) return "one-sweep step: the basis has more rows than the fused one-sweep form takes (1520)";
  if (!one_sweep_fused_applies(h, n) || !full_fused)
    return "one-sweep step: needs one rank, fused-norm full re-orthogonalisation and a matrix with 5 or 7 entries per row (the fused one-sweep form)";
  if (j < 2) return "one-sweep step: need j >= 2";
  if (form == 1) return j + 1 > n ? "one-sweep step: need j < n" : nullptr;
  if (form == 2)
    return j + 2 > n || qtw_ldp(n + 1) > kOneSweepPairMaxLdp ? "one-sweep step: a pair needs j + 2 <= n and n + 1 within the pair walk's run length"
                                                              : nullptr;
  if (form == 4)
    return j + 4 > n || os_quad_ldp(n - 4) > os_quad_max_ldp() ? "one-sweep step: a group needs j + 4 <= n and n within the group walk's run length"
                                                               : nullptr;
  return "one-sweep step: form must be 1, 2 or 4";
}
static int one_sweep_step_blocks(lz_handle h, int form, bool wide) {
  return form == 4 ? os_quad_sweep_blocks(h->rows_pad, wide) : form == 2 ? os_pair_sweep_blocks(h->rows_pad, wide) : os_sweep_blocks(h->rows_pad);
}
int one_sweep_state_set(lz_handle h, int j, const double* G, const double* H, const double* chat, double alpha_prev, double beta_prev,
                        double beta_prev2) {
  const int n = h->n;
  if (const char* why = one_sweep_step_refusal(h, n, j, 1)) return fail(h, LZ_ERR_STATE, why);
  OneSweepState st;
  int blocks = 0;
  for (int wide = 0; wide < 2; ++wide)
    blocks = std::max({blocks, os_pair_sweep_blocks(h->rows_pad, wide != 0), 2 * os_quad_sweep_blocks(h->rows_pad, wide != 0)});
  LZ_TRY(one_sweep_setup(h, n, st, blocks));
  const size_t nn = (size_t)n * n * sizeof(double);
  LZ_HIP(h, hipMemcpyAsync(st.G, G, nn, hipMemcpyHostToDevice, h->stream));
  LZ_HIP(h, hipMemcpyAsync(st.H, H, nn, hipMemcpyHostToDevice, h->stream));
  LZ_HIP(h, hipMemcpyAsync(st.chat, chat, (size_t)j * sizeof(double), hipMemcpyHostToDevice, h->stream));
  LZ_HIP(h, hipMemcpyAsync(h->d_alpha + (j - 1), &alpha_prev, sizeof(double), hipMemcpyHostToDevice, h->stream));
  LZ_HIP(h, hipMemcpyAsync(h->d_beta + (j - 2), &beta_prev, sizeof(double), hipMemcpyHostToDevice, h->stream));
  if (j >= 3) LZ_HIP(h, hipMemcpyAsync(h->d_beta + (j - 3), &beta_prev2, sizeof(double), hipMemcpyHostToDevice, h->stream));
  LZ_HIP(h, hipStreamSynchronize(h->stream));
  h->os_step_n = n;
  return LZ_OK;
}
int one_sweep_step_run(lz_handle h, int form, int j, bool wide, int* blocks) {
  const int n = h->n;
  if (const char* why = one_sweep_step_refusal(h, n, j, form)) return fail(h, LZ_ERR_STATE, why);
  if (h->os_step_n != n || !h->d_os) return fail(h, LZ_ERR_STATE, "one-sweep step: no state set for this basis (lz_os_state_set after lz_basis_alloc)");
  OneSweepState st;
  one_sweep_view(h, n, st);
  const int nb = one_sweep_step_blocks(h, form, wide);
  const int pairs = h->last_os_pairs, quads = h->last_os_quads;
  const size_t tap = (size_t)nb * (form == 4 ? 4 * os_quad_ldp(j) : form == 2 ? 2 * os_pair_ldp(j) : qtw_ldp(j + 2));
  if (h->tap_cap < tap) {
    LZ_TRY(dev_alloc(h, h->d_tap, tap));
    h->tap_cap = tap;
  }
  h->tap_count = tap;
  h->tap_what = form == 4 ? "one-sweep group walk" : form == 2 ? "one-sweep pair walk" : "one-sweep";
  int rc;
  if (form == 4) {
    rc = one_sweep_quad_iter(h, n, j, st, nb, wide);
  } else if (form == 2) {
    rc = one_sweep_pair_iter(h, n, j, st, nb, wide);
  } else {
    begin_iter(h, j);
    rc = one_sweep_fused_iter(h, n, j, st);
  }
  h->tap_what = nullptr;
  h->last_os_pairs = pairs;
  h->last_os_quads = quads;
  LZ_TRY(rc);
  LZ_HIP(h, hipStreamSynchronize(h->stream));
  if (blocks) *blocks = nb;
  return LZ_OK;
}
int one_sweep_state_get(lz_handle h, int form, int j, double* G, double* H, double* chat, double* g, double* gq, double* d, double* elog,
                        double* alpha, double* beta, double* nrm2, double* r2, int* ist, int* ldg, int* ldp) {
  const int n = h->n;
  if (h->os_step_n != n || !h->d_os) return fail(h, LZ_ERR_STATE, "one-sweep step: no state set for this basis (lz_os_state_set after lz_basis_alloc)");
  OneSweepState st;
  one_sweep_view(h, n, st);
  auto get = [&](void* dst, const void* src, size_t bytes) {
    return dst ? hipMemcpyAsync(dst, src, bytes, hipMemcpyDeviceToHost, h->stream) : hipSuccess;
  };
  const size_t nn = (size_t)n * n * sizeof(double);
  LZ_HIP(h, get(G, st.G, nn));
  LZ_HIP(h, get(H, st.H, nn));
  LZ_HIP(h, get(chat, st.chat, ((size_t)n + 1) * sizeof(double)));
  LZ_HIP(h, get(g, st.g, ((size_t)2 * n + 2) * sizeof(double)));
  LZ_HIP(h, get(gq, st.gq, (size_t)4 * (n + 4) * sizeof(double)));
  LZ_HIP(h, get(d, h->d_c, ((size_t)4 * qtw_ldp(n + 2) + 16) * sizeof(double)));
  LZ_HIP(h, get(elog, st.elog, ((size_t)n + 1) * sizeof(double)));
  LZ_HIP(h, get(alpha, h->d_alpha, ((size_t)n + 1) * sizeof(double)));
  LZ_HIP(h, get(beta, h->d_beta, ((size_t)n + 1) * sizeof(double)));
  LZ_HIP(h, get(nrm2, h->d_nrm2, sizeof(double)));
  LZ_HIP(h, get(r2, h->d_r2, (size_t)h->rows * sizeof(double)));
  LZ_HIP(h, get(ist, h->d_osi, 8 * sizeof(int)));
  LZ_HIP(h, hipStreamSynchronize(h->stream));
  if (ldg) *ldg = n + 4;
  if (ldp) *ldp = form == 4 ? os_quad_ldp(j) : form == 2 ? os_pair_ldp(j) : qtw_ldp(j + 2);
  return LZ_OK;
}

int one_sweep_raw_get(lz_handle h, int j0, int count, double* rows, double* part, int64_t part_count) {
  if (rows) {
    if (count < 1 || j0 < 0 || j0 + count > h->n) return fail(h, LZ_ERR_ARG, "lz_os_raw_get: rows out of range");
    LZ_HIP(h, hipMemcpy2DAsync(rows, (size_t)h->rows_pad * sizeof(double), h->d_V + (int64_t)j0 * h->ldv, (size_t)h->ldv * sizeof(double),
                               (size_t)h->rows_pad * sizeof(double), (size_t)count, hipMemcpyDeviceToHost, h->stream));
  }
  if (part) {
    if (part_count < 0 || (size_t)part_count > h->tap_count || !h->d_tap) return fail(h, LZ_ERR_STATE, "lz_os_raw_get: the last step's walk left fewer partials");
    LZ_HIP(h, hipMemcpyAsync(part, h->d_tap, (size_t)part_count * sizeof(double), hipMemcpyDeviceToHost, h->stream));
  }
  LZ_HIP(h, hipStreamSynchronize(h->stream));
  return LZ_OK;
}

enum Loop {
  LOOP_SIX = 0,
  LOOP_SMALL_ENGINE = 1,
  LOOP_FUSED_SMALL = 2,
  LOOP_THREE_TERM_FUSED = 3,
  LOOP_SMALL_STEP = 4,
  LOOP_ONE_REDUCE_REPEATED = 5,
  LOOP_ONE_REDUCE = 6,
  LOOP_PARTIAL_DEVICE = 7,
  LOOP_PARTIAL_ONE_REDUCE = 8,
  LOOP_ONE_SWEEP = 9
};

Loop choose_loop(lz_handle h, int n, const QtwPlan* plan = nullptr) {
  const int f = h->flags;
  const QtwPlan& qp = plan ? *plan : h->qplan;
  const bool default_kernels = qp.family == 2 && !(f & (LZ_FLAG_QTW_MFMA | LZ_FLAG_QTW_VALU)) && h->tune[1] == 0 && h->tune[8] == 0;
  const bool full_fused = (f & LZ_FLAG_FUSED_NORM) && !(f & LZ_FLAG_REORTH_PARTIAL);
  if ((f & LZ_FLAG_ONE_REDUCE) && !(f & LZ_FLAG_REORTH_PARTIAL) && qp.family == 2) return LOOP_ONE_REDUCE;
  if ((f & LZ_FLAG_ONE_REDUCE) && (f & LZ_FLAG_REORTH_PARTIAL) && default_kernels && h->tune[18] != 1 && !(f & LZ_FLAG_OVERLAP_HALO))
    return LOOP_PARTIAL_ONE_REDUCE;
  if ((f & LZ_FLAG_REORTH_PARTIAL) && default_kernels && h->tune[18] != 1 && !(f & LZ_FLAG_OVERLAP_HALO)) return LOOP_PARTIAL_DEVICE;
  const bool one_rank = h->world == 1 && h->comm_kind == 0;
#ifdef LZ_KBENCH
  const bool want_steps = h->tune[15] == 5 && n <= kSmallStepMaxN;
  if ((h->tune[15] == 2 || h->tune[15] == 3 || want_steps) && one_rank && full_fused && default_kernels && !(f & LZ_FLAG_SPMV_SCALAR) &&
      qp.L == 512 && h->rows_pad <= kSmallMaxPadRows && n <= kSmallMaxPadRows && small_engine_applies(h))
    return want_steps ? LOOP_SMALL_STEP : LOOP_SMALL_ENGINE;
  const bool knob_auto = h->tune[15] == 0 || h->tune[15] == 5;
#else
  const bool knob_auto = h->tune[15] == 0;
#endif
  const bool one_sweep_ok = one_rank && full_fused && default_kernels && !(f & LZ_FLAG_OVERLAP_HALO) && n >= 2 && n <= kOneSweepMaxN;
  if (h->tune[15] >= 6 && h->tune[15] <= 11 && one_sweep_ok) return LOOP_ONE_SWEEP;
  if (!knob_auto || !full_fused || !default_kernels) return LOOP_SIX;
  if (one_rank && qp.G <= 8 && n <= 4096 && h->part_cap >= fused_coff(h) + (size_t)(n + 16) * (size_t)qp.G) return LOOP_FUSED_SMALL;
  if (!(f & LZ_FLAG_OVERLAP_HALO) && h->rows_pad <= kThreeTermFusedMaxRows) return LOOP_THREE_TERM_FUSED;
  if (one_sweep_ok) return LOOP_ONE_SWEEP;
  return LOOP_SIX;
}

struct HostOmega {
  static constexpr double eps = 2.220446049250313e-16, thresh = 1.4901161193847656e-08;
  std::vector<double> w_prev, w_cur, w_new, ha, hb;
  double normA = 0.0;
  bool force_next = false;
  void start(int n, double nrm2_0) {
    for (auto* v : {&w_prev, &w_cur, &w_new, &ha, &hb}) v->assign((size_t)n + 1, 0.0);
    w_cur[0] = 1.0;
    hb[0] = std::sqrt(nrm2_0);
  }
  bool due(int j) {
    bool over = false;
    if (j >= 1) {
      std::fill(w_new.begin(), w_new.end(), 0.0);
      w_new[(size_t)j] = 1.0;
      w_new[(size_t)j - 1] = eps;
      double worst = 0.0;
      for (int k = 0; k + 2 <= j; ++k) {
        double t = hb[(size_t)k + 1] * w_cur[(size_t)k + 1] + (ha[(size_t)k] - ha[(size_t)j - 1]) * w_cur[(size_t)k] -
                   hb[(size_t)j - 1] * w_prev[(size_t)k];
        if (k > 0) t += hb[(size_t)k] * w_cur[(size_t)k - 1];
        t += (t < 0 ? -1.0 : 1.0) * 2.0 * eps * normA;
        w_new[(size_t)k] = t / hb[(size_t)j];
        worst = std::max(worst, std::fabs(w_new[(size_t)k]));
      }
      over = worst > thresh;
      std::swap(w_prev, w_cur);
      std::swap(w_cur, w_new);
    }
    const bool sweep = (j == 0) || over || force_next;
    force_next = over;
    if (sweep)
      for (int k = 0; k < j; ++k) w_cur[(size_t)k] = eps;
    return sweep;
  }
  void feed(int j, double alpha, double nrm2) {
    ha[(size_t)j] = alpha;
    hb[(size_t)j + 1] = std::sqrt(nrm2);
    normA = std::max(normA, std::fabs(alpha) + hb[(size_t)j] + hb[(size_t)j + 1]);
  }
};

static int read_back_step(lz_handle h, int j) {
  if (!h->h_pinned) LZ_HIP(h, hipHostMalloc(reinterpret_cast<void**>(&h->h_pinned), 8 * sizeof(double), hipHostMallocDefault));
  if (j >= 0) LZ_HIP(h, hipMemcpyAsync(&h->h_pinned[0], h->d_alpha + j, sizeof(double), hipMemcpyDeviceToHost, h->stream));
  LZ_HIP(h, hipMemcpyAsync(&h->h_pinned[1], h->d_nrm2, sizeof(double), hipMemcpyDeviceToHost, h->stream));
  LZ_HIP(h, hipStreamSynchronize(h->stream));
  h->host_syncs += 1;
  return LZ_OK;
}

int run_loop_six(lz_handle h, int n, int j0 = 0) {
  const bool partial = (h->flags & LZ_FLAG_REORTH_PARTIAL) != 0;
  const bool fused = (h->flags & LZ_FLAG_FUSED_NORM) != 0 && !partial;
  if (j0 == 0) {
    LZ_TRY(warm_up(h, !fused));
  } else if (!fused) {
    LZ_HIP(h, hipMemsetAsync(h->d_c + n, 0, sizeof(double), h->stream));
    LZ_TRY(step_three_term(h, 0, -1, h->d_c + n, nullptr, true));
  }
  HostOmega omega;
  if (partial) {
    LZ_TRY(read_back_step(h, -1));
    omega.start(n, h->h_pinned[1]);
  }
  int sweeps = 0;
  for (int j = j0; j < n; ++j) {
    begin_iter(h, j);
    const int bidx = beta_index(n, j);
    double* bslot = h->d_beta + bidx;
    if (!partial || omega.due(j)) {
      ++sweeps;
      LZ_TRY(step_reorth(h, j, j + 1, true, bidx, true));
    } else {
      Scope sc(h, LZ_K_QTW, 16.0 * (double)h->rows, (double)h->rows);
      launch_scale_store(basis_row(h, j), h->d_r, h->d_nrm2, bslot, h->rows_pad, h->stream);
      LZ_TRY(check_launch(h, "scale_store"));
    }
    LZ_TRY(step_spmv(h, j));
    LZ_TRY(step_three_term(h, j, j > 0 ? j - 1 : -1, h->d_alpha + j, bslot, !fused));
    if (partial) {
      LZ_TRY(read_back_step(h, j));
      omega.feed(j, h->h_pinned[0], h->h_pinned[1]);
    }
  }
  h->last_sweeps = sweeps;
  h->r_state = 1;
  return LZ_OK;
}

int run_loop_partial_device(lz_handle h, int n, int j0 = 0, const double* state_j0 = nullptr) {
  const double M = (double)h->rows;
  if (h->om_n < n) {
    LZ_TRY(dev_alloc(h, h->d_om, omega_state_doubles(n)));
    LZ_TRY(dev_alloc(h, h->d_omi, omega_state_ints(n) + 1));
    h->om_n = n;
  }
  h->om_run_n = n;
  if (j0 > 0) {
    std::vector<double> st(omega_state_doubles(n), 0.0);
    st[0] = state_j0[0];
    st[1] = state_j0[1];
    const double* hb_s = state_j0 + 2;
    const double* W_s = hb_s + (j0 + 2);
    double* hb_d = st.data() + 2;
    double* W_d = hb_d + (n + 2);
    for (int k = 0; k < j0 + 2; ++k) hb_d[k] = hb_s[k];
    for (int r = 0; r < 3; ++r)
      for (int k = 0; k <= j0; ++k) W_d[(size_t)r * (n + 1) + k] = W_s[(size_t)r * (j0 + 1) + k];
    LZ_HIP(h, hipMemcpyAsync(h->d_om, st.data(), st.size() * sizeof(double), hipMemcpyHostToDevice, h->stream));
    LZ_HIP(h, hipMemsetAsync(h->d_omi, 0, (omega_state_ints(n) + 1) * sizeof(int), h->stream));
    LZ_HIP(h, hipStreamSynchronize(h->stream));
  }
  LZ_HIP(h, hipMemsetAsync(h->d_omi + omega_state_ints(n), 0, sizeof(int), h->stream));
  const int* gate = h->d_omi;
  const bool one_rank = h->world <= 1 && !(h->tune[6] && h->comm_kind);
  if (one_rank && h->kind == 1 && h->tune[18] != 2 && h->tune[17] != 1 && !h->csr.ell_rb && !h->csr.pb &&
      (h->csr.fixed_k == 5 || h->csr.fixed_k == 7))
    LZ_HIP(h, ell_build(h->csr, 0, h->stream));
  const bool fuse_scale = one_rank && h->kind == 1 && ell_usable(h->csr, h->flags) && h->tune[18] != 2;
  if (j0 == 0) LZ_TRY(step_spmv(h, 0));
  int np = 0;
  auto three_term_and_decide = [&](int j, int jm1, const double* d_alpha, const double* d_beta, double* r, bool decide, int jn) -> int {
    LZ_TRY(step_three_term(h, j, jm1, d_alpha, d_beta, false, &np, r));
    Scope sc(h, LZ_K_FINAL, 0, 0);
    if (one_rank && decide) {
      launch_omega(h->d_part, np, h->d_nrm2, h->d_alpha, jn, n, h->d_om, h->d_omi, h->stream);
      return check_launch(h, "final_sum(nrm2) + omega");
    }
    launch_final_sum(h->d_part, np, h->d_nrm2, h->stream);
    LZ_TRY(check_launch(h, "final_sum(nrm2)"));
    LZ_TRY(comm_allreduce(h, h->d_nrm2, 1));
    if (decide) {
      launch_omega(nullptr, 0, h->d_nrm2, h->d_alpha, jn, n, h->d_om, h->d_omi, h->stream, h->d_c);
      LZ_TRY(check_launch(h, "omega"));
    }
    return LZ_OK;
  };
  if (j0 > 0) LZ_HIP(h, hipMemsetAsync(h->d_c + n, 0, sizeof(double), h->stream));
  LZ_TRY(three_term_and_decide(0, -1, j0 > 0 ? h->d_c + n : h->d_alpha, nullptr, h->d_r, true, j0));
  double* rcur = h->d_r;
  double* rnext = h->d_r2;
  for (int j = j0; j < n; ++j) {
    begin_iter(h, j);
    double* bslot = beta_slot(h, n, j);
    {
// ... 482 lines not shown
```

### lanczos_amd/csrc/lz_reorth.hip

```cpp
#include <algorithm>
#include <cmath>
#include <type_traits>

#include "lz_device.h"

namespace lz {

constexpr int kFinalThreads = 1024;
__device__ __forceinline__ double final_sum_1024(const double* __restrict__ part, int n, double* sm) {
  double a0 = 0.0, a1 = 0.0, a2 = 0.0, a3 = 0.0;
  int i = threadIdx.x;
  for (; i + 3 * kFinalThreads < n; i += 4 * kFinalThreads) {
    a0 += part[i];
    a1 += part[i + kFinalThreads];
    a2 += part[i + 2 * kFinalThreads];
    a3 += part[i + 3 * kFinalThreads];
  }
  for (; i < n; i += kFinalThreads) a0 += part[i];
  const double acc = wave_sum((a0 + a1) + (a2 + a3));
  const int lane = threadIdx.x & 63, w = threadIdx.x >> 6;
  if (lane == 0) sm[w] = acc;
  __syncthreads();
  double t = 0.0;
  if (threadIdx.x == 0) {
// ... 948 lines not shown
      hipLaunchKernelGGL((k_update<true, 1, 8>), dim3(grid), dim3(kTPB), 0, s, V, ldv, p0, n2, nrows, j, c, r_fused, beta);
    else
      hipLaunchKernelGGL((k_update<false, 1, 8>), dim3(grid), dim3(kTPB), 0, s, V, ldv, p0, n2, nrows, j, c, r_fused, beta);
    return;
  }
  const int64_t span = n2 - p0;
  int P = variant == 3 ? 8 : (variant == 4 ? 4 : 0);
  if (!P) {
    double best = -1.0;
    P = 2;
    for (int cand : {16, 8, 4, 2}) {
      const int64_t G = (span + (int64_t)kTPB * cand - 1) / ((int64_t)kTPB * cand);
      const double g = (double)G / kNumCU, bal = g / std::ceil(g);
      if (bal >= 0.93) {
        P = cand;
        break;
      }
      if (bal > best) {
        best = bal;
        P = cand;
      }
    }
  }
  if (variant == 6 || (variant == 0 && P == 16 && span > 16384)) {
    if (r_fused) launch_update_slice<true, 16, 1>(V, ldv, p0, n2, nrows, j, c, r_fused, beta, raw_c, s, 0, 0, cG, cldp, gate, usub, asub);
    else launch_update_slice<false, 16, 1>(V, ldv, p0, n2, nrows, j, c, r_fused, beta, 0, s, 0, 0, 0, 0, gate);
    return;
  }
  if (variant == 0 && span <= 4096 && r_fused && nrows > 64 && pos_hi < 0 && pos_lo <= 0 && !gate) {
    const int grid_e = (int)((len + kTPB - 1) / kTPB);
    hipLaunchKernelGGL(k_update_elem, dim3(grid_e), dim3(kTPB), raw_c == 2 ? (size_t)nrows * sizeof(double) : 0, s, V, ldv, len, nrows, j, c, r_fused,
                       beta, raw_c, cG, cldp);
    return;
  }
  if ((variant == 0 && span <= 16384) || variant == 5) {
    if (r_fused) launch_update_slice<true, 1, 32>(V, ldv, p0, n2, nrows, j, c, r_fused, beta, raw_c, s, pos_lo_b, pos_hi_b, cG, cldp, gate, usub, asub);
    else launch_update_slice<false, 1, 32>(V, ldv, p0, n2, nrows, j, c, r_fused, beta, 0, s, pos_lo_b, pos_hi_b, 0, 0, gate);
  } else if (P == 8) {
    if (r_fused) launch_update_slice<true, 8, 2>(V, ldv, p0, n2, nrows, j, c, r_fused, beta, raw_c, s, 0, 0, cG, cldp, gate, usub, asub);
    else launch_update_slice<false, 8, 2>(V, ldv, p0, n2, nrows, j, c, r_fused, beta, 0, s, 0, 0, 0, 0, gate);
  } else if (P == 4) {
    if (r_fused) launch_update_slice<true, 4, 4>(V, ldv, p0, n2, nrows, j, c, r_fused, beta, raw_c, s, 0, 0, cG, cldp, gate, usub, asub);
    else launch_update_slice<false, 4, 4>(V, ldv, p0, n2, nrows, j, c, r_fused, beta, 0, s, 0, 0, 0, 0, gate);
  } else {
    if (r_fused) launch_update_slice<true, 2, 8>(V, ldv, p0, n2, nrows, j, c, r_fused, beta, raw_c, s, 0, 0, cG, cldp, gate, usub, asub);
    else launch_update_slice<false, 2, 8>(V, ldv, p0, n2, nrows, j, c, r_fused, beta, 0, s, 0, 0, 0, 0, gate);
  }
}

__global__ __launch_bounds__(kTPB) void k_scale_store(double* __restrict__ vj, const double* __restrict__ r,
                                                     const double* __restrict__ nrm2, double* __restrict__ beta_slot, int64_t n2,
                                                     const int* __restrict__ gate) {
  if (gate && gate[0] != 0) return;
  const double beta = sqrt(nrm2[0]);
  if (blockIdx.x == 0 && threadIdx.x == 0) beta_slot[0] = beta;
  const double2* r2 = reinterpret_cast<const double2*>(r);
  double2* v2 = reinterpret_cast<double2*>(vj);
  for (int64_t i = (int64_t)blockIdx.x * kTPB + threadIdx.x; i < n2; i += (int64_t)gridDim.x * kTPB) {
    double2 x = r2[i];
    x.x = x.x / beta;
    x.y = x.y / beta;
    v2[i] = x;
  }
}
void launch_scale_store(double* vj, const double* r, const double* nrm2, double* beta_slot, int64_t len, hipStream_t s, const int* gate) {
  const int64_t n2 = len >> 1;
  int64_t g = (n2 + kTPB - 1) / kTPB;
  if (g > 4096) g = 4096;
  if (g < 1) g = 1;
  hipLaunchKernelGGL(k_scale_store, dim3((int)g), dim3(kTPB), 0, s, vj, r, nrm2, beta_slot, n2, gate);
}

__global__ void k_fused_prepare(double* __restrict__ c, int j, double* __restrict__ beta_slot) {
  const double rr = c[j];
  const double b = sqrt(rr);
  for (int i = threadIdx.x; i < j; i += blockDim.x) c[i] = c[i] / b;
  __syncthreads();
  if (threadIdx.x == 0) {
    c[j] = rr / (b * b);
    beta_slot[0] = b;
  }
}
__global__ void k_onereduce_prepare(double* __restrict__ buf, int m, int ldp, double* __restrict__ alpha_slot, double* __restrict__ bad,
                                    double* __restrict__ beta_prev, double* __restrict__ uu_keep) {
  const double uu = buf[ldp + m];
  const double a = buf[ldp + m + 2] / uu;
  for (int i = threadIdx.x; i < m; i += blockDim.x) buf[i] = buf[i] - a * buf[ldp + i];
  __syncthreads();
  if (threadIdx.x == 0) {
    const double rr = buf[m], ur = buf[ldp + m + 1];
    const double v = (rr - 2.0 * a * ur) + a * a * uu;
    if (!(v > 1e-4 * rr)) bad[0] = 1.0;
    buf[m] = v;
    alpha_slot[0] = a;
    if (beta_prev) beta_prev[0] = beta_prev[0] * sqrt(uu / uu_keep[0]);
    uu_keep[0] = uu;
  }
}
void launch_onereduce_prepare(double* buf, int m, int ldp, double* alpha_slot, double* bad, double* beta_prev, double* uu_keep, hipStream_t s) {
  hipLaunchKernelGGL(k_onereduce_prepare, dim3(1), dim3(kTPB), 0, s, buf, m, ldp, alpha_slot, bad, beta_prev, uu_keep);
}
__global__ void k_onereduce_finish(const double* __restrict__ buf, int ldp, double* __restrict__ alpha_last, double* __restrict__ beta_last,
                                   const double* __restrict__ uu_keep) {
  if (threadIdx.x == 0) {
    const double uu = buf[ldp];
    alpha_last[0] = buf[ldp + 2] / uu;
    if (beta_last) beta_last[0] = beta_last[0] * sqrt(uu / uu_keep[0]);
  }
}
void launch_onereduce_finish(const double* buf, int ldp, double* alpha_last, double* beta_last, const double* uu_keep, hipStream_t s) {
  hipLaunchKernelGGL(k_onereduce_finish, dim3(1), dim3(64), 0, s, buf, ldp, alpha_last, beta_last, uu_keep);
}

void launch_fused_prepare(double* c, int j, double* beta_slot, hipStream_t s) {
  hipLaunchKernelGGL(k_fused_prepare, dim3(1), dim3(kTPB), 0, s, c, j, beta_slot);
}

__global__ __launch_bounds__(kTPB) void k_three_term(double* __restrict__ r, const double* __restrict__ vj,
                                                    const double* __restrict__ vjm1, const double* __restrict__ alpha,
                                                    const double* __restrict__ beta, int64_t n2, double* __restrict__ part) {
  __shared__ double sm[kTPB / 64];
  const double a = alpha[0];
  const double b = vjm1 ? beta[0] : 0.0;
  double2* r2 = reinterpret_cast<double2*>(r);
  const double2* v2 = reinterpret_cast<const double2*>(vj);
  const double2* m2 = reinterpret_cast<const double2*>(vjm1);
  double acc = 0.0;
  for (int64_t i = (int64_t)blockIdx.x * kTPB + threadIdx.x; i < n2; i += (int64_t)gridDim.x * kTPB) {
    double2 x = r2[i];
    const double2 v = ld_stream<1>(v2 + i);
    x.x = x.x - v.x * a;
    x.y = x.y - v.y * a;
    if (vjm1) {
      const double2 m = ld_stream<1>(m2 + i);
      x.x = x.x - m.x * b;
      x.y = x.y - m.y * b;
    }
    r2[i] = x;
    acc = fma(x.x, x.x, acc);
    acc = fma(x.y, x.y, acc);
  }
  acc = block_sum(acc, sm);
  if (threadIdx.x == 0) part[blockIdx.x] = acc;
}

int launch_three_term(double* r, const double* vj, const double* vjm1, const double* alpha, const double* beta,
                      int64_t len, double* part, hipStream_t s) {
  const int64_t n2 = len >> 1;
  int64_t g = (n2 + kTPB - 1) / kTPB;
  if (g > 2048) g = 2048;
  if (g < 1) g = 1;
  hipLaunchKernelGGL(k_three_term, dim3((int)g), dim3(kTPB), 0, s, r, vj, vjm1, alpha, beta, n2, part);
  return (int)g;
}

__global__ __launch_bounds__(kTPB) void k_three_term_self(double* __restrict__ r, const double* __restrict__ u, const double* __restrict__ vm,
                                                         const double* __restrict__ beta, int64_t n2, double* __restrict__ part) {
  __shared__ double sm[kTPB / 64];
  const double b = vm ? beta[0] : 0.0;
  double2* r2 = reinterpret_cast<double2*>(r);
  const double2* u2 = reinterpret_cast<const double2*>(u);
  const double2* m2 = reinterpret_cast<const double2*>(vm);
  double s0 = 0.0, s1 = 0.0, s2 = 0.0;
  for (int64_t i = (int64_t)blockIdx.x * kTPB + threadIdx.x; i < n2; i += (int64_t)gridDim.x * kTPB) {
    double2 x = r2[i];
    const double2 uu = u2[i];
    if (vm) {
      const double2 m = ld_stream<1>(m2 + i);
      x.x = x.x - m.x * b;
      x.y = x.y - m.y * b;
      r2[i] = x;
    }
    s0 = fma(x.x, x.x, s0);
    s0 = fma(x.y, x.y, s0);
    s1 = fma(uu.x, x.x, s1);
    s1 = fma(uu.y, x.y, s1);
    s2 = fma(uu.x, uu.x, s2);
    s2 = fma(uu.y, uu.y, s2);
  }
  s0 = block_sum(s0, sm);
  s1 = block_sum(s1, sm);
  s2 = block_sum(s2, sm);
  if (threadIdx.x == 0) {
    part[blockIdx.x] = s0;
    part[gridDim.x + blockIdx.x] = s1;
    part[2 * gridDim.x + blockIdx.x] = s2;
  }
}
int launch_three_term_self(double* r, const double* u, const double* vm, const double* beta, int64_t len, double* part, hipStream_t s) {
  const int64_t n2 = len >> 1;
  int64_t g = (n2 + kTPB - 1) / kTPB;
  if (g > 2048) g = 2048;
  if (g < 1) g = 1;
  hipLaunchKernelGGL(k_three_term_self, dim3((int)g), dim3(kTPB), 0, s, r, u, vm, beta, n2, part);
  return (int)g;
}

__global__ __launch_bounds__(kTPB) void k_gather(const double* __restrict__ x, const int32_t* __restrict__ idx, int64_t n,
                                                double* __restrict__ buf) {
  const int64_t i = (int64_t)blockIdx.x * kTPB + threadIdx.x;
  if (i < n) buf[i] = x[idx[i]];
}
void launch_gather(const double* x, const int32_t* idx, int64_t n, double* buf, hipStream_t s) {
  if (n <= 0) return;
  hipLaunchKernelGGL(k_gather, dim3((int)((n + kTPB - 1) / kTPB)), dim3(kTPB), 0, s, x, idx, n, buf);
}

template <int P, int RU, int MODE>
__global__ __launch_bounds__(kTPB) void k_os_sweep(double* __restrict__ V, int64_t ldv, int64_t n2, int j, const double* __restrict__ coef,
                                                  const double* __restrict__ r, const double* __restrict__ nrm2,
                                                  double* __restrict__ beta_slot, int ldp, double* __restrict__ part,
                                                  const int* __restrict__ gate, double* __restrict__ dst,
                                                  const double* __restrict__ alpha_prev, const double* __restrict__ beta_prev) {
  if (MODE == 1 && gate[0] == 0) return;
  extern __shared__ double keep[];
  const int lane = threadIdx.x & 63, wv = threadIdx.x >> 6;
  const int64_t base = (int64_t)blockIdx.x * (kTPB * P) + threadIdx.x;
  const int64_t ld2 = ldv >> 1;
  const double2* V2 = reinterpret_cast<const double2*>(V);
  double2* out = reinterpret_cast<double2*>(dst);
  using pos_t = std::conditional_t<MODE == 2, int, int64_t>;
  pos_t pos[P];
  bool ok[P];
#pragma unroll
  for (int p = 0; p < P; ++p) {
    pos[p] = (pos_t)(base + (int64_t)p * kTPB);
    ok[p] = base + (int64_t)p * kTPB < n2;
    if (!ok[p]) pos[p] = (pos_t)(n2 - 1);
  }
  double2 w[P];
  double b = 1.0, cs = MODE == 2 ? 1.0 : 0.0;
  if (MODE == 0) {
    const double s2 = nrm2[0];
    b = sqrt(s2);
    cs = s2 / (b * b);
    if (blockIdx.x == 0 && threadIdx.x == 0) beta_slot[0] = b;
  }
  double tx[P], ty[P];
#pragma unroll
  for (int p = 0; p < P; ++p) tx[p] = ty[p] = 0.0;
  if (MODE == 2) {
    const double a = alpha_prev[0];
    const bool two = j >= 2;
    const double bp = two ? beta_prev[0] : 0.0;
    const double c1 = coef[j - 1], c2 = two ? coef[j - 2] : 0.0;
    const double2* y2 = reinterpret_cast<const double2*>(r);
    const double2* v1 = V2 + (int64_t)(j - 1) * ld2;
    const double2* v2 = V2 + (int64_t)(two ? j - 2 : 0) * ld2;
    double d1 = 0.0, d2 = 0.0, ww = 0.0;
    constexpr int PB = P < 8 ? P : 8;
    auto batches = [&](auto two_c) {
      constexpr bool TWO = decltype(two_c)::value;
#pragma unroll
      for (int p0 = 0; p0 < P; p0 += PB) {
        double2 x[PB], v[PB], m[PB];
#pragma unroll
        for (int q = 0; q < PB; ++q) {
          x[q] = y2[pos[p0 + q]];
          v[q] = ld_stream<1>(v1 + pos[p0 + q]);
          m[q] = TWO ? ld_stream<1>(v2 + pos[p0 + q]) : make_double2(0.0, 0.0);
        }
#pragma unroll
        for (int q = 0; q < PB; ++q) {
          const int p = p0 + q;
          x[q].x = x[q].x - v[q].x * a;
          x[q].y = x[q].y - v[q].y * a;
          if (TWO) {
            x[q].x = x[q].x - m[q].x * bp;
            x[q].y = x[q].y - m[q].y * bp;
          }
          if (!ok[p]) x[q] = make_double2(0.0, 0.0);
          w[p] = x[q];
          ww = fma(x[q].x, x[q].x, ww);
          ww = fma(x[q].y, x[q].y, ww);
          d1 = fma(v[q].x, x[q].x, d1);
          d1 = fma(v[q].y, x[q].y, d1);
          tx[p] = tx[p] + c1 * v[q].x;
          ty[p] = ty[p] + c1 * v[q].y;
          if (TWO) {
            d2 = fma(m[q].x, x[q].x, d2);
            d2 = fma(m[q].y, x[q].y, d2);
            tx[p] = tx[p] + c2 * m[q].x;
            ty[p] = ty[p] + c2 * m[q].y;
          }
        }
        __builtin_amdgcn_sched_barrier(0);
      }
    };
    if (two)
      batches(std::true_type());
    else
      batches(std::false_type());
    ww = wave_sum(ww);
    d1 = wave_sum(d1);
    d2 = wave_sum(d2);
    if (lane == 0) {
      keep[wv * ldp + j + 1] = ww;
      keep[wv * ldp + j - 1] = d1;
      if (two) keep[wv * ldp + j - 2] = d2;
    }
  } else {
#pragma unroll
    for (int p = 0; p < P; ++p) {
      if (MODE == 0) {
        w[p] = reinterpret_cast<const double2*>(r)[pos[p]];
        w[p].x = w[p].x / b;
// ... 92 lines not shown
                    const double* beta_prev) {
  const int64_t n2 = len >> 1;
  const int P = os_sweep_p(n2);
  const int grid = (int)((n2 + (int64_t)kTPB * P - 1) / ((int64_t)kTPB * P));
  const int ldp = qtw_ldp(mode == 2 ? j + 2 : j + 1);
  const size_t lds = mode != 1 ? (size_t)(kTPB / 64) * ldp * sizeof(double) : 0;
  if (!dst) dst = V + (int64_t)j * ldv;
#define LZ_OS_ARGS V, ldv, n2, j, coef, r, nrm2, beta_slot, ldp, part, gate, dst, alpha_prev, beta_prev
#define LZ_OS_GO(PP, RR)                                                                                       \
  do {                                                                                                         \
    if (mode == 0)                                                                                             \
      hipLaunchKernelGGL((k_os_sweep<PP, RR, 0>), dim3(grid), dim3(kTPB), lds, s, LZ_OS_ARGS);                 \
    else if (mode == 2)                                                                                        \
      hipLaunchKernelGGL((k_os_sweep<PP, RR, 2>), dim3(grid), dim3(kTPB), lds, s, LZ_OS_ARGS);                 \
    else                                                                                                       \
      hipLaunchKernelGGL((k_os_sweep<PP, RR, 1>), dim3(grid), dim3(kTPB), lds, s, LZ_OS_ARGS);                 \
  } while (0)
  switch (P) {
    case 16: LZ_OS_GO(16, 1); break;
    case 8: LZ_OS_GO(8, 2); break;
    case 4: LZ_OS_GO(4, 4); break;
    case 2: LZ_OS_GO(2, 8); break;
    default: LZ_OS_GO(1, 16); break;
  }
#undef LZ_OS_GO
#undef LZ_OS_ARGS
  return grid;
}

constexpr int kOsCB = 4;
template <class RowA, class VecB, class Len, class F>
__device__ __forceinline__ void os_wave_dots(int count, RowA rowa, VecB vecb, Len len, F f) {
  const int lane = threadIdx.x & 63, wv = threadIdx.x >> 6, nw = blockDim.x >> 6;
  for (int i0 = wv * kOsCB; i0 < count; i0 += nw * kOsCB) {
    double acc[kOsCB];
    const double* ra[kOsCB];
    int m = 0;
#pragma unroll
    for (int q = 0; q < kOsCB; ++q) {
      const int i = i0 + q < count ? i0 + q : count - 1;
      acc[q] = 0.0;
      ra[q] = rowa(i);
      m = max(m, len(i));
    }
#pragma unroll 4
    for (int l = lane; l < m; l += 64) {
      const double b = vecb(l);
#pragma unroll
      for (int q = 0; q < kOsCB; ++q) {
        const int i = i0 + q < count ? i0 + q : count - 1;
        acc[q] = fma(l < len(i) ? ra[q][l] : 0.0, b, acc[q]);
      }
    }
#pragma unroll
    for (int q = 0; q < kOsCB; ++q) {
      const double t = wave_sum(acc[q]);
      if (lane == 0 && i0 + q < count) f(i0 + q, t);
    }
  }
}

template <bool FUSED>
__global__ __launch_bounds__(kFinalThreads) void k_os_post(const double* __restrict__ d, const double* __restrict__ chat, double* __restrict__ G,
                                                          double* __restrict__ H, int n, int j, double* __restrict__ nrm2, double tau,
                                                          double* __restrict__ g, int* __restrict__ ist, double* __restrict__ elog) {
  extern __shared__ double smem[];
  double* col = smem;
  double* sc = col + (j + 1);
  double* sd = sc + (j + 1);
  __shared__ double smax[kFinalThreads / 64];
  __shared__ int s_trip;
  const double s2 = FUSED ? d[j + 1] : nrm2[0];
  const double b = sqrt(s2), cs = FUSED ? 1.0 : s2 / (b * b);
  double em = 0.0;
  for (int i = threadIdx.x; i < j; i += blockDim.x) {
    const double di = FUSED ? d[i] / b : d[i], ci = FUSED ? chat[i] / b : chat[i];
    const double e = fabs(di - ci);
    em = e == e ? fmax(em, e) : __builtin_inf();
    sd[i] = di;
    sc[i] = ci;
  }
  if (threadIdx.x == 0) {
    col[j] = FUSED ? d[j] / s2 : d[j];
    if (FUSED) nrm2[0] = s2;
  }
#pragma unroll
  for (int off = 32; off > 0; off >>= 1) em = fmax(em, __shfl_down(em, off, 64));
  if ((threadIdx.x & 63) == 0) smax[threadIdx.x >> 6] = em;
  __syncthreads();
  os_wave_dots(
      j, [&](int i) { return G + (int64_t)i * n; }, [&](int l) { return sc[l]; }, [&](int) { return j; },
      [&](int i, double t) { col[i] = (2.0 - cs) * sd[i] - t; });
  if (threadIdx.x == 0) {
    double m = 0.0;
    for (int k = 0; k < (int)(blockDim.x >> 6); ++k) m = fmax(m, smax[k]);
    const int trip = (j > 0 && !(m <= tau)) ? 1 : 0;
    s_trip = trip;
    elog[j] = m;
    ist[0] = trip;
    ist[1] += trip;
  }
  __syncthreads();
  const int trip = s_trip;
  if (trip) {
    for (int i = threadIdx.x; i < j; i += blockDim.x) g[i] = col[i];
    __syncthreads();
    os_wave_dots(
        j, [&](int i) { return G + (int64_t)i * n; }, [&](int l) { return g[l]; }, [&](int) { return j; },
        [&](int i, double t) {
          col[i] = g[i] - t;
          sd[i] = g[i] * (t - 2.0 * g[i]);
        });
    __syncthreads();
    if (threadIdx.x == 0) {
      double vv = col[j];
      for (int i = 0; i < j; ++i) vv += sd[i];
      col[j] = vv;
    }
    if (FUSED)
      for (int i = threadIdx.x; i < j; i += blockDim.x) g[n + i] = b * g[i];
    __syncthreads();
  }
  for (int i = threadIdx.x; i <= j; i += blockDim.x) {
    G[(int64_t)j * n + i] = col[i];
    G[(int64_t)i * n + j] = col[i];
  }
  if (j > 0) {
    const double f = b / (2.0 - cs);
    double* hc = H + (int64_t)(j - 1) * n;
    for (int l = threadIdx.x; l < j; l += blockDim.x) {
      const double c = trip ? sc[l] + g[l] : sc[l];
      hc[l] = hc[l] + f * c;
    }
    if (threadIdx.x == 0) hc[j] = f;
  }
}

void launch_os_post(const double* d, const double* chat, double* G, double* H, int n, int j, double* nrm2, double tau, double* g, int* ist,
                    double* elog, bool fused, hipStream_t s) {
  const size_t lds = (size_t)3 * (j + 1) * sizeof(double);
  if (fused)
    hipLaunchKernelGGL(k_os_post<true>, dim3(1), dim3(kFinalThreads), lds, s, d, chat, G, H, n, j, nrm2, tau, g, ist, elog);
  else
    hipLaunchKernelGGL(k_os_post<false>, dim3(1), dim3(kFinalThreads), lds, s, d, chat, G, H, n, j, nrm2, tau, g, ist, elog);
}

template <bool FUSED>
__global__ __launch_bounds__(kFinalThreads) void k_os_sum_predict(const double* __restrict__ part, int np, double* __restrict__ sum_out,
                                                                 const double* __restrict__ G, double* __restrict__ H, int n, int j,
                                                                 const double* __restrict__ alpha_j, const double* __restrict__ beta_j,
                                                                 double* __restrict__ chat, int predict) {
  __shared__ double sm[kFinalThreads / 64];
  __shared__ double s_sum;
  const double t = final_sum_1024(part, np, sm);
  if (threadIdx.x == 0) {
    sum_out[0] = t;
    s_sum = t;
  }
  if (!predict) return;
  __syncthreads();
  const double a = FUSED ? s_sum : alpha_j[0], bj = j > 0 ? beta_j[0] : 0.0, bn = FUSED ? 1.0 : sqrt(s_sum);
  const double* gj = G + (int64_t)j * n;
  const double* gm = G + (int64_t)(j > 0 ? j - 1 : 0) * n;
  auto finish = [&](int i, double s) {
    s = s - a * gj[i];
    if (j > 0) s = s - bj * gm[i];
    chat[i] = s / bn;
  };
  os_wave_dots(
      j, [&](int i) { return H + (int64_t)i * n; }, [&](int l) { return gj[l]; }, [&](int i) { return i + 2; }, finish);
  if (threadIdx.x == 0) finish(j, a);
  double* hc = H + (int64_t)j * n;
  for (int l = threadIdx.x; l < n; l += blockDim.x) hc[l] = l == j ? a : (l == j - 1 ? bj : 0.0);
}

void launch_os_sum_predict(const double* part, int np, double* sum_out, const double* G, double* H, int n, int j, const double* alpha_j,
                           const double* beta_j, double* chat, bool fused, bool predict, hipStream_t s) {
  if (fused)
    hipLaunchKernelGGL(k_os_sum_predict<true>, dim3(1), dim3(kFinalThreads), 0, s, part, np, sum_out, G, H, n, j, alpha_j, beta_j, chat, predict ? 1 : 0);
  else
    hipLaunchKernelGGL(k_os_sum_predict<false>, dim3(1), dim3(kFinalThreads), 0, s, part, np, sum_out, G, H, n, j, alpha_j, beta_j, chat, predict ? 1 : 0);
}

__global__ __launch_bounds__(kFinalThreads) void k_os_pair_predict(const double* __restrict__ part, int np, double* __restrict__ alpha_out,
                                                                  const double* __restrict__ nrm2, const double* __restrict__ chat,
                                                                  const double* __restrict__ G, double* __restrict__ H, int n, int j,
                                                                  double* __restrict__ kap, double* __restrict__ pout) {
  extern __shared__ double smem[];
  double* cn = smem;
  double* gp = cn + (j + 1);
  double* q = gp + (j + 1);
  double* mu = q + (j + 1);
  double* red = mu + (j + 1);
  __shared__ double sm[kFinalThreads / 64];
  __shared__ double s_a0, s_cq;
  const double t0 = final_sum_1024(part, np, sm);
  if (threadIdx.x == 0) {
    alpha_out[0] = t0;
    s_a0 = t0;
  }
  const double b = sqrt(nrm2[0]);
  double* hc = H + (int64_t)(j - 1) * n;
  for (int i = threadIdx.x; i < j; i += blockDim.x) {
    const double ci = chat[i] / b;
    cn[i] = ci;
    hc[i] = hc[i] + b * ci;
  }
  if (threadIdx.x == 0) {
    hc[j] = b;
    cn[j] = 0.0;
    gp[j] = 1.0;
  }
  __syncthreads();
  const double a0 = s_a0;
  os_wave_dots(
      j, [&](int i) { return G + (int64_t)i * n; }, [&](int l) { return cn[l]; }, [&](int) { return j; },
      [&](int i, double t) { gp[i] = cn[i] - t; });
  os_wave_dots(
      j, [&](int i) { return (const double*)(H + (int64_t)i * n); }, [&](int l) { return cn[l]; }, [&](int i) { return min(i + 2, j); },
      [&](int i, double t) { q[i] = i == j - 1 ? t + b : t; });
  {
    const int Lp = (j + 1 + 63) & ~63, nchunk = kFinalThreads / Lp;
    const int l = threadIdx.x % Lp, ch = threadIdx.x / Lp;
    if (ch < nchunk) {
      double acc = 0.0;
      if (l <= j) {
        int i = ch;
        if (i < l - 1) i += (l - 1 - i + nchunk - 1) / nchunk * nchunk;
        for (; i < j; i += nchunk) acc = fma(H[(int64_t)i * n + l], cn[i], acc);
      }
      red[ch * Lp + l] = acc;
    }
    __syncthreads();
    if (threadIdx.x <= j) {
      double m = 0.0;
      for (int c = 0; c < nchunk; ++c) m += red[c * Lp + threadIdx.x];
      mu[threadIdx.x] = m;
    }
  }
  __syncthreads();
  if (threadIdx.x < 64) {
    double acc = 0.0;
    for (int i = threadIdx.x; i < j; i += 64) acc = fma(cn[i], q[i], acc);
    acc = wave_sum(acc);
    if (threadIdx.x == 0) s_cq = acc;
  }
  __syncthreads();
  const double* gm = G + (int64_t)(j - 1) * n;
  os_wave_dots(
      j, [&](int i) { return (const double*)(H + (int64_t)i * n); }, [&](int l) { return gp[l]; }, [&](int i) { return i + 2; },
      [&](int i, double t) {
        const double pi = (t - a0 * gp[i]) - b * gm[i];
        pout[i] = pi;
        kap[i] = (mu[i] - a0 * cn[i]) + pi;
      });
  if (threadIdx.x == 0) {
    const double vAv = a0 - 2.0 * s_cq;
    const double pj = (vAv - a0 * gp[j]) - b * gp[j - 1];
    pout[j] = pj;
    kap[j] = mu[j] + pj;
  }
}

void launch_os_pair_predict(const double* part, int np, double* alpha_out, const double* nrm2, const double* chat, const double* G, double* H,
                            int n, int j, double* kap, double* p, hipStream_t s) {
  const size_t lds = ((size_t)4 * (j + 1) + kFinalThreads) * sizeof(double);
  hipLaunchKernelGGL(k_os_pair_predict, dim3(1), dim3(kFinalThreads), lds, s, part, np, alpha_out, nrm2, chat, G, H, n, j, kap, p);
}

template <int P, int RU>
__global__ __launch_bounds__(kTPB) void k_os_pair_sweep(const double* __restrict__ V, double* __restrict__ vj, int64_t ldv, int n2, int j,
                                                       const double* __restrict__ chat, const double* __restrict__ kap,
                                                       const double* __restrict__ wbuf, double* __restrict__ ybuf,
                                                       const double* __restrict__ nrm2, const double* __restrict__ alpha0, int ldp,
                                                       double* __restrict__ part) {
  extern __shared__ double keep[];
  const int lane = threadIdx.x & 63, wv = threadIdx.x >> 6;
  const int64_t base = (int64_t)blockIdx.x * (kTPB * P) + threadIdx.x;
  const int64_t ld2 = ldv >> 1;
  const double2* V2 = reinterpret_cast<const double2*>(V);
  double2* y2 = reinterpret_cast<double2*>(ybuf);
  double* kw = keep + wv * 2 * ldp;
  int pos[P];
  bool ok[P];
#pragma unroll
  for (int p = 0; p < P; ++p) {
    ok[p] = base + (int64_t)p * kTPB < n2;
    pos[p] = ok[p] ? (int)(base + (int64_t)p * kTPB) : n2 - 1;
  }
  const double b = sqrt(nrm2[0]), a0 = alpha0[0];
  double2 w[P], z[P];
  double tx[P], ty[P], sx[P], sy[P];
  {
    const double c1 = chat[j - 1], k1 = kap[j - 1];
    const double2* w2 = reinterpret_cast<const double2*>(wbuf);
    const double2* v1 = V2 + (int64_t)(j - 1) * ld2;
    double d1 = 0.0, d2 = 0.0;
    constexpr int PB = P < 8 ? P : 8;
#pragma unroll
    for (int p0 = 0; p0 < P; p0 += PB) {
      double2 x[PB], y[PB], m[PB];
#pragma unroll
      for (int q = 0; q < PB; ++q) {
        x[q] = w2[pos[p0 + q]];
        y[q] = y2[pos[p0 + q]];
        m[q] = ld_stream<1>(v1 + pos[p0 + q]);
      }
#pragma unroll
      for (int q = 0; q < PB; ++q) {
        const int p = p0 + q;
        double2 zz;
        zz.x = (y[q].x - a0 * (x[q].x / b)) - b * m[q].x;
        zz.y = (y[q].y - a0 * (x[q].y / b)) - b * m[q].y;
        if (!ok[p]) {
          x[q] = make_double2(0.0, 0.0);
          zz = make_double2(0.0, 0.0);
        }
        w[p] = x[q];
        z[p] = zz;
        d1 = fma(m[q].x, x[q].x, d1);
        d1 = fma(m[q].y, x[q].y, d1);
        d2 = fma(m[q].x, zz.x, d2);
        d2 = fma(m[q].y, zz.y, d2);
        tx[p] = c1 * m[q].x;
        ty[p] = c1 * m[q].y;
        sx[p] = k1 * m[q].x;
        sy[p] = k1 * m[q].y;
      }
      __builtin_amdgcn_sched_barrier(0);
    }
    d1 = wave_sum(d1);
// ... 125 lines not shown
    if ((threadIdx.x & 63) == 0) dst[threadIdx.x >> 6] = em;
  };
  double em = 0.0;
  for (int i = threadIdx.x; i < j; i += blockDim.x) {
    const double di = d[i] / b, ci = chat[i] / b;
    const double e = fabs(di - ci);
    em = e == e ? fmax(em, e) : __builtin_inf();
    dn[i] = di;
    cn[i] = ci;
    kp[i] = kap[i];
  }
  if (threadIdx.x == 0) {
    kp[j] = kap[j];
    colj[j] = uu / s2;
  }
  wave_max(em, smax[0]);
  __syncthreads();
  os_wave_dots(
      j, [&](int i) { return (const double*)(G + (int64_t)i * n); }, [&](int l) { return cn[l]; }, [&](int) { return j; },
      [&](int i, double t) { colj[i] = dn[i] - t; });
  __syncthreads();
  os_wave_dots(
      j, [&](int i) { return (const double*)(G + (int64_t)i * n); }, [&](int l) { return kp[l]; }, [&](int) { return j; },
      [&](int i, double t) { col2[i] = (d[ldp + i] - (t + colj[i] * kp[j])) / b2; });
  if (threadIdx.x < 64) {
    double acc = 0.0;
    for (int l = threadIdx.x; l < j; l += 64) acc = fma(colj[l], kp[l], acc);
    acc = wave_sum(acc);
    if (threadIdx.x == 0) col2[j] = (vz - (acc + colj[j] * kp[j])) / b2;
  }
  __syncthreads();
  em = 0.0;
  for (int i = threadIdx.x; i <= j; i += blockDim.x) {
    const double e = fabs(col2[i]);
    em = e == e ? fmax(em, e) : __builtin_inf();
  }
  wave_max(em, smax[1]);
  for (int i = threadIdx.x; i <= j; i += blockDim.x) {
    G[(int64_t)j * n + i] = colj[i];
    G[(int64_t)i * n + j] = colj[i];
    G[(int64_t)(j + 1) * n + i] = col2[i];
    G[(int64_t)i * n + j + 1] = col2[i];
  }
  double* hc = H + (int64_t)j * n;
  for (int l = threadIdx.x; l < n; l += blockDim.x) {
    double v = l <= j ? pin[l] : 0.0;
    if (l == j - 1) v = b + v;
    if (l == j) v = a0 + v;
    if (l == j + 1) v = b2;
    hc[l] = v;
  }
  __syncthreads();
  if (threadIdx.x == 0) {
    double m1 = 0.0, m2 = 0.0;
    for (int k = 0; k < (int)(blockDim.x >> 6); ++k) {
      m1 = fmax(m1, smax[0][k]);
      m2 = fmax(m2, smax[1][k]);
    }
    G[(int64_t)(j + 1) * n + j + 1] = 1.0;
    nrm2[0] = uu2;
    elog[j] = m1;
    elog[j + 1] = m2;
    if (!(m1 <= tau) || !(m2 <= tau) || !(b2 == b2)) ist[3] = 1;
  }
}

void launch_os_pair_post(const double* d, int ldp, const double* chat, const double* kap, const double* p, double* G, double* H, int n, int j,
                         double* nrm2, const double* alpha_j, double tau, int* ist, double* elog, hipStream_t s) {
  const size_t lds = ((size_t)2 * j + (size_t)3 * (j + 1)) * sizeof(double);
  hipLaunchKernelGGL(k_os_pair_post, dim3(1), dim3(kFinalThreads), lds, s, d, ldp, chat, kap, p, G, H, n, j, nrm2, alpha_j, tau, ist, elog);
}

__global__ __launch_bounds__(kFinalThreads) void k_os_quad_predict(const double* __restrict__ part, int np, double* __restrict__ nrm2,
                                                                  const double* __restrict__ chat, const double* __restrict__ G,
                                                                  const double* __restrict__ H, int n, int j, const double* __restrict__ alpha,
                                                                  const double* __restrict__ beta, double* __restrict__ gout, int ldg) {
  extern __shared__ double smem[];
  const int L = j + 4;
  __shared__ double sm[kFinalThreads / 64];
  __shared__ double s_n;
  const double t0 = final_sum_1024(part, np, sm);
  if (threadIdx.x == 0) {
    nrm2[0] = t0;
    s_n = t0;
  }
  __syncthreads();
  const double b[4] = {beta[0], beta[1], beta[2], sqrt(s_n)};
  const double a[3] = {alpha[0], alpha[1], alpha[2]};
  for (int i = threadIdx.x; i < 4 * L; i += blockDim.x) smem[i] = i < j ? chat[i] / b[0] : 0.0;
  __syncthreads();
  const double* gm = G + (int64_t)(j - 1) * n;
#pragma unroll
  for (int t = 0; t < 3; ++t) {
    const double* gt = smem + t * L;
    const double* gp = t ? smem + (t - 1) * L : gm;
    double* gn = smem + (t + 1) * L;
    os_wave_dots(
        j, [&](int i) { return H + (int64_t)i * n; }, [&](int l) { return gt[l]; }, [&](int i) { return min(i + 2, j); },
        [&](int i, double s) {
          if (i == j - 1) s = s + b[0] * (t ? gt[j] : 1.0);
          gn[i] = ((s - a[t] * gt[i]) - b[t] * gp[i]) / b[t + 1];
        });
    if (threadIdx.x == 0) {
      for (int s = 0; s < t; ++s) {
        const double up = s + 1 == t ? 1.0 : gt[j + s + 1];
        const double lo = s ? gt[j + s - 1] : gt[j - 1];
        const double pv = s == t - 1 ? 1.0 : gp[j + s];
        gn[j + s] = ((((b[s + 1] * up + a[s] * gt[j + s]) + b[s] * lo) - a[t] * gt[j + s]) - b[t] * pv) / b[t + 1];
      }
      const double lo = t ? gt[j + t - 1] : gt[j - 1];
      gn[j + t] = -(b[t] * lo) / b[t + 1];
    }
    __syncthreads();
  }
  for (int i = threadIdx.x; i < 4 * L; i += blockDim.x) gout[(i / L) * ldg + i % L] = smem[i];
}

void launch_os_quad_predict(const double* part, int np, double* nrm2, const double* chat, const double* G, const double* H, int n, int j,
                            const double* alpha, const double* beta, double* gout, int ldg, hipStream_t s) {
  const size_t lds = (size_t)4 * (j + 4) * sizeof(double);
  hipLaunchKernelGGL(k_os_quad_predict, dim3(1), dim3(kFinalThreads), lds, s, part, np, nrm2, chat, G, H, n, j, alpha, beta, gout, ldg);
}

template <int NV>
__device__ __forceinline__ double quad_joint_sum(double (&v)[NV], int lane) {
  int off = 32;
#pragma unroll
  for (int cnt = NV; cnt > 1; cnt >>= 1, off >>= 1) {
    const bool hi = (lane & off) != 0;
#pragma unroll
    for (int i = 0; i < cnt / 2; ++i) {
      const double send = hi ? v[i] : v[i + cnt / 2];
      const double mine = hi ? v[i + cnt / 2] : v[i];
      v[i] = mine + __shfl_xor(send, off, 64);
    }
  }
#pragma unroll
  for (; off > 0; off >>= 1) v[0] = v[0] + __shfl_xor(v[0], off, 64);
  return v[0];
}
template <int NV>
__device__ __forceinline__ int quad_slot(int lane) {
  int idx = 0, off = 32;
#pragma unroll
  for (int cnt = NV; cnt > 1; cnt >>= 1, off >>= 1)
    if (lane & off) idx += cnt / 2;
  return idx;
}
template <int NV>
__device__ __forceinline__ bool quad_writer(int lane) { return (lane & (64 / NV - 1)) == 0; }

template <int P, int RU>
__global__ __launch_bounds__(kTPB) void k_os_quad_sweep(double* __restrict__ V, int64_t ldv, int n2, int j, const double* __restrict__ g, int ldg,
                                                       const double* __restrict__ zbuf, const double* __restrict__ nrm2, int ldp,
                                                       double* __restrict__ part) {
  extern __shared__ double keep[];
  constexpr int NV = 4 * RU;
  const int lane = threadIdx.x & 63, wv = threadIdx.x >> 6;
  const int64_t base = (int64_t)blockIdx.x * (kTPB * P) + threadIdx.x;
  const int64_t ld2 = ldv >> 1;
  double2* V2 = reinterpret_cast<double2*>(V);
  double* kw = keep + wv * 4 * ldp;
  int pos[P];
  bool ok[P];
#pragma unroll
  for (int p = 0; p < P; ++p) {
    ok[p] = base + (int64_t)p * kTPB < n2;
    pos[p] = ok[p] ? (int)(base + (int64_t)p * kTPB) : n2 - 1;
  }
  const double b3 = sqrt(nrm2[0]);
  double2 x[4][P];
  double sx[4][P], sy[4][P];
  {
    const double2* z2 = reinterpret_cast<const double2*>(zbuf);
#pragma unroll
    for (int p = 0; p < P; ++p) {
#pragma unroll
      for (int t = 0; t < 3; ++t) x[t][p] = V2[(int64_t)(j + t) * ld2 + pos[p]];
      const double2 zz = z2[pos[p]];
      x[3][p] = make_double2(zz.x / b3, zz.y / b3);
#pragma unroll
      for (int t = 0; t < 4; ++t) {
        if (!ok[p]) x[t][p] = make_double2(0.0, 0.0);
        sx[t][p] = 0.0;
        sy[t][p] = 0.0;
      }
    }
  }
  const int slot = quad_slot<NV>(lane), su = slot >> 2, st = slot & 3;
  const bool writer = quad_writer<NV>(lane);
  for (int k = 0; k < j; k += RU) {
    double2 q[RU][P];
#pragma unroll
    for (int u = 0; u < RU; ++u)
      if (k + u < j) {
        const double2* row = V2 + (int64_t)(k + u) * ld2;
#pragma unroll
        for (int p = 0; p < P; ++p) q[u][p] = ld_stream<1>(row + pos[p]);
      }
    double d[NV];
#pragma unroll
    for (int u = 0; u < RU; ++u) {
#pragma unroll
      for (int t = 0; t < 4; ++t) d[u * 4 + t] = 0.0;
      if (k + u < j) {
#pragma unroll
        for (int t = 0; t < 4; ++t) {
          const double c = g[t * ldg + k + u];
          double dd = 0.0;
#pragma unroll
          for (int p = 0; p < P; ++p) {
            sx[t][p] = fma(c, q[u][p].x, sx[t][p]);
            sy[t][p] = fma(c, q[u][p].y, sy[t][p]);
            dd = fma(q[u][p].x, x[t][p].x, dd);
            dd = fma(q[u][p].y, x[t][p].y, dd);
          }
          d[u * 4 + t] = dd;
        }
      }
    }
    const double tot = quad_joint_sum<NV>(d, lane);
    if (writer && k + su < j) kw[st * ldp + k + su] = tot;
  }
  double gi[4][4];
#pragma unroll
  for (int t = 1; t < 4; ++t)
#pragma unroll
    for (int s = 0; s < t; ++s) gi[t][s] = g[t * ldg + j + s];
  double mm[4][4], vv[4];
#pragma unroll
  for (int t = 0; t < 4; ++t) {
    vv[t] = 0.0;
#pragma unroll
    for (int s = 0; s < 4; ++s) mm[t][s] = 0.0;
  }
#pragma unroll
  for (int p = 0; p < P; ++p) {
    double2 v[4];
#pragma unroll
    for (int t = 0; t < 4; ++t) {
      v[t] = make_double2(x[t][p].x - sx[t][p], x[t][p].y - sy[t][p]);
#pragma unroll
      for (int s = 0; s < t; ++s) {
        v[t].x = v[t].x - gi[t][s] * v[s].x;
        v[t].y = v[t].y - gi[t][s] * v[s].y;
      }
    }
    if (ok[p]) {
#pragma unroll
      for (int t = 0; t < 4; ++t) {
        st_stream<1>(V2 + (int64_t)(j + t) * ld2 + pos[p], v[t]);
        vv[t] = fma(v[t].x, v[t].x, vv[t]);
        vv[t] = fma(v[t].y, v[t].y, vv[t]);
#pragma unroll
        for (int s = 0; s < t; ++s) {
          mm[t][s] = fma(v[s].x, x[t][p].x, mm[t][s]);
          mm[t][s] = fma(v[s].y, x[t][p].y, mm[t][s]);
        }
      }
    }
  }
#pragma unroll
  for (int t = 0; t < 4; ++t) {
    const double a = wave_sum(vv[t]);
    if (lane == 0) kw[t * ldp + j + t] = a;
#pragma unroll
    for (int s = 0; s < t; ++s) {
      const double m = wave_sum(mm[t][s]);
      if (lane == 0) kw[t * ldp + j + s] = m;
    }
  }
  __syncthreads();
  double* mine = part + (int64_t)blockIdx.x * (4 * ldp);
  for (int i = threadIdx.x; i < 4 * ldp; i += kTPB) {
    const bool used = i % ldp <= j + i / ldp;
    const double t = used ? ((keep[i] + keep[4 * ldp + i]) + keep[8 * ldp + i]) + keep[12 * ldp + i] : 0.0;
    __builtin_nontemporal_store(t, mine + i);
  }
}

static int os_quad_sweep_p(int64_t n2, bool wide8) {
  const int P = os_sweep_p(n2);
  return P >= 8 ? (wide8 ? 8 : 4) : P;
}
int os_quad_sweep_blocks(int64_t len, bool wide8) {
  const int64_t n2 = len >> 1;
  const int P = os_quad_sweep_p(n2, wide8);
  return (int)((n2 + (int64_t)kTPB * P - 1) / ((int64_t)kTPB * P));
}
int os_quad_ldp(int j) { return qtw_ldp(j + 4); }

int launch_os_quad_sweep(double* V, int64_t ldv, int64_t len, int j, const double* g, int ldg, const double* z, const double* nrm2, double* part,
                         bool wide8, hipStream_t s) {
  const int64_t n2 = len >> 1;
  const int P = os_quad_sweep_p(n2, wide8);
  const int grid = (int)((n2 + (int64_t)kTPB * P - 1) / ((int64_t)kTPB * P));
  const int ldp = os_quad_ldp(j);
  const size_t lds = os_quad_lds_bytes(ldp);
#define LZ_OSQ_GO(PP, RR) \
  hipLaunchKernelGGL((k_os_quad_sweep<PP, RR>), dim3(grid), dim3(kTPB), lds, s, V, ldv, (int)n2, j, g, ldg, z, nrm2, ldp, part)
  switch (P) {
    case 8: LZ_OSQ_GO(8, 1); break;
    case 4: LZ_OSQ_GO(4, 2); break;
    case 2: LZ_OSQ_GO(2, 4); break;
    default: LZ_OSQ_GO(1, 4); break;
  }
#undef LZ_OSQ_GO
  return grid;
}

__global__ __launch_bounds__(kFinalThreads) void k_os_quad_post(const double* __restrict__ d, int ldp, const double* __restrict__ gin, int ldg,
                                                               double* __restrict__ G, double* __restrict__ H, int n, int j,
                                                               const double* __restrict__ nrm2, const double* __restrict__ alpha,
                                                               double* __restrict__ beta, double tau, int* __restrict__ ist,
                                                               double* __restrict__ elog) {
  extern __shared__ double smem[];
  const int L = j + 6;
  double* C = smem;
  double* col = C + 4 * L;
  double* hn = col + 4 * L;
  double* red = hn + 4 * L;
  __shared__ double smax[2][kFinalThreads / 64];
  __shared__ double s_in[6];
  const double b[4] = {beta[0], beta[1], beta[2], sqrt(nrm2[0])};
  const double a[3] = {alpha[0], alpha[1], alpha[2]};
  const int lane = threadIdx.x & 63, wv = threadIdx.x >> 6;
  auto wave_max = [&](double em, double* dst) {
#pragma unroll
    for (int off = 32; off > 0; off >>= 1) em = fmax(em, __shfl_down(em, off, 64));
    if (lane == 0) dst[wv] = em;
  };
  double e_old = 0.0, e_in = 0.0;
  for (int i = threadIdx.x; i < 4 * L; i += blockDim.x) {
    const int t = i / L, r = i % L;
    double c = 0.0;
    if (r < j + t) {
      c = gin[t * ldg + r];
      const double e = fabs(d[t * ldp + r] - c);
      if (r < j)
        e_old = e == e ? fmax(e_old, e) : __builtin_inf();
      else
        e_in = e == e ? fmax(e_in, e) : __builtin_inf();
    } else if (r == j + t) {
      c = 1.0;
    }
    C[i] = c;
    col[i] = 0.0;
    hn[i] = 0.0;
  }
  wave_max(e_old, smax[0]);
  wave_max(e_in, smax[1]);
  __syncthreads();
#pragma unroll 1
  for (int t = 0; t < 4; ++t) {
    const double* Ct = C + t * L;
    double* ct = col + t * L;
    os_wave_dots(
        j, [&](int i) { return (const double*)(G + (int64_t)i * n); }, [&](int l) { return Ct[l]; }, [&](int) { return j; },
        [&](int i, double s) { ct[i] = d[t * ldp + i] - s; });
  }
  __syncthreads();
#pragma unroll 1
  for (int t = 0; t < 4; ++t) {
    const double* Ct = C + t * L;
    double* ct = col + t * L;
    for (int i = threadIdx.x; i < j; i += blockDim.x) {
      double v = ct[i];
      for (int s = 0; s < t; ++s) v = v - col[s * L + i] * Ct[j + s];
      ct[i] = v;
    }
    if (wv < t) {
      const double* cs = col + wv * L;
      double acc = 0.0;
      for (int l = lane; l < j; l += 64) acc = fma(cs[l], Ct[l], acc);
      acc = wave_sum(acc);
      if (lane == 0) s_in[wv] = acc;
    }
    __syncthreads();
    if (threadIdx.x == 0) {
      for (int s = 0; s < t; ++s) {
        double v = d[t * ldp + j + s] - s_in[s];
        for (int q = 0; q < t; ++q) v = v - col[max(s, q) * L + j + min(s, q)] * Ct[j + q];
        ct[j + s] = v;
      }
      ct[j + t] = d[t * ldp + j + t];
    }
    __syncthreads();
  }
  {
    const int Lp = (j + 63) & ~63, nchunk = kFinalThreads / Lp;
    const int l = threadIdx.x % Lp, ch = threadIdx.x / Lp;
#pragma unroll 1
    for (int t = 0; t < 3; ++t) {
      const double* Ct = C + t * L;
      if (ch < nchunk) {
        double acc = 0.0;
        if (l < j) {
          int i = ch;
          if (i < l - 1) i += (l - 1 - i + nchunk - 1) / nchunk * nchunk;
          for (; i < j - 1; i += nchunk) acc = fma(H[(int64_t)i * n + l], Ct[i], acc);
        }
        red[ch * Lp + l] = acc;
      }
      __syncthreads();
      if (threadIdx.x < j) {
        double m = 0.0;
        for (int c = 0; c < nchunk; ++c) m += red[c * Lp + threadIdx.x];
        hn[(1 + t) * L + threadIdx.x] = m;
      }
      __syncthreads();
    }
  }
  {
    const double* hc = H + (int64_t)(j - 1) * n;
    for (int l = threadIdx.x; l <= j; l += blockDim.x) hn[l] = l < j ? hc[l] + b[0] * C[l] : b[0];
  }
  __syncthreads();
#pragma unroll 1
  for (int t = 0; t < 3; ++t) {
    const double* Ct = C + t * L;
    const double* Cn = C + (t + 1) * L;
    double* ht = hn + (1 + t) * L;
    for (int l = threadIdx.x; l <= j + t + 1; l += blockDim.x) {
      double sub = ht[l] + Ct[j - 1] * hn[l];
      for (int s = 0; s < t; ++s) sub = sub + Ct[j + s] * hn[(1 + s) * L + l];
      const double last = t ? b[t] * C[(t - 1) * L + l] : (l == j - 1 ? b[0] : 0.0);
      ht[l] = ((b[t + 1] * Cn[l] + a[t] * Ct[l]) + last) - sub;
    }
    __syncthreads();
  }
  for (int i = threadIdx.x; i < 4 * L; i += blockDim.x) {
    const int t = i / L, r = i % L;
    if (r <= j + t) {
      G[(int64_t)(j + t) * n + r] = col[i];
      G[(int64_t)r * n + j + t] = col[i];
    }
  }
  for (int l = threadIdx.x; l <= j; l += blockDim.x) H[(int64_t)(j - 1) * n + l] = hn[l];
  for (int i = threadIdx.x; i < 3 * n; i += blockDim.x) {
    const int t = i / n, l = i % n;
    H[(int64_t)(j + t) * n + l] = l <= j + t + 1 ? hn[(1 + t) * L + l] : 0.0;
  }
  if (threadIdx.x == 0) {
    double m1 = 0.0, m2 = 0.0;
    for (int k = 0; k < (int)(blockDim.x >> 6); ++k) {
      m1 = fmax(m1, smax[0][k]);
      m2 = fmax(m2, smax[1][k]);
    }
    beta[3] = b[3];
    const double m = fmax(m1, m2);
    for (int t = 0; t < 4; ++t) elog[j + t] = m;
    if (!(m1 <= tau) || !(m2 <= tau) || !(b[3] == b[3])) ist[4] = 1;
  }
// ... 15 lines not shown
```

Before: 1926.

## Chain unnormalized three-term vectors in quad group and overlap post on side stream

```diff
diff --git a/lanczos_amd/csrc/lz_api.hip b/lanczos_amd/csrc/lz_api.hip
--- a/lanczos_amd/csrc/lz_api.hip
+++ b/lanczos_amd/csrc/lz_api.hip
@@ -113,7 +113,7 @@
 }
 }
 
-Scope::Scope(lz_handle h_, int cls_, double bytes, double flops) : h(h_), cls(cls_) {
+Scope::Scope(lz_handle h_, int cls_, double bytes, double flops, hipStream_t stream) : h(h_), cls(cls_), st(stream ? stream : h_->stream) {
   if (roctx_on()) {
     g_roctx.push(kClassNames[cls]);
     marked = true;
@@ -135,13 +135,13 @@
         return;
       }
     }
-    hipEventRecord(a, h->stream);
+    hipEventRecord(a, st);
   }
 }
 Scope::~Scope() {
   if (marked) g_roctx.pop();
   if (on) {
-    hipEventRecord(b, h->stream);
+    hipEventRecord(b, st);
     h->events.push_back({cls, a, b});
   }
 }
@@ -433,6 +433,7 @@
   if (!h) return LZ_OK;
   hipSetDevice(h->dev);
   hipStreamSynchronize(h->stream);
+  if (h->os_stream) hipStreamSynchronize(h->os_stream);
   if (h->comm && g_rccl.CommDestroy) g_rccl.CommDestroy(h->comm);
   big_free(h->csr.rowptr);
   big_free(h->csr.colidx);
@@ -470,6 +471,14 @@
   big_free(h->d_xfull);
   big_free(h->d_om);
   big_free(h->d_os);
+  big_free(h->d_ospart);
+  if (h->os_stream) {
+    hipStreamSynchronize(h->os_stream);
+    hipStreamDestroy(h->os_stream);
+    hipEventDestroy(h->e_os_walk);
+    hipEventDestroy(h->e_os_alpha);
+    hipEventDestroy(h->e_os_ready);
+  }
   big_free(h->d_osi);
   big_free(h->d_tap);
   big_free(h->d_omi);
@@ -525,11 +534,11 @@
 
 int lz_set_tuning(lz_handle h, int index, int value) {
   if (!h) return LZ_ERR_ARG;
-  if (index < 0 || index >= 24) return fail(h, LZ_ERR_ARG, "lz_set_tuning: knob index out of range");
+  if (index < 0 || index >= kTuneKnobs) return fail(h, LZ_ERR_ARG, "lz_set_tuning: knob index out of range");
   if ((index == 1 && value >= 20) || (index == 3 && value != 0) || (index == 9 && value >= 10))
     return fail(h, LZ_ERR_ARG, "lz_set_tuning: the timing-only ablation arms were removed in round 5 (their measurements are in profiles/)");
 #ifndef LZ_KBENCH
-  if ((index == 15 && value >= 2 && (value < 6 || value > 11)) || (index == 9 && value >= 2) || (index == 11 && value >= 2) || (index == 22 && value >= 2))
+  if ((index == 15 && value >= 2 && (value < 6 || value > 13)) || (index == 9 && value >= 2) || (index == 11 && value >= 2) || (index == 22 && value >= 2))
     return fail(h, LZ_ERR_ARG, "lz_set_tuning: this A/B arm was retired from the product library (build with KBENCH=1)");
 #endif
   if (value < 0) return fail(h, LZ_ERR_ARG, "lz_set_tuning: negative value");
diff --git a/lanczos_amd/csrc/lz_context.h b/lanczos_amd/csrc/lz_context.h
--- a/lanczos_amd/csrc/lz_context.h
+++ b/lanczos_amd/csrc/lz_context.h
@@ -169,13 +169,15 @@
   int iters = 0, cycles = 0, done = 0;
 };
 
+constexpr int kTuneKnobs = 24;
+
 struct lz_context {
   int dev = 0;
   hipStream_t stream = nullptr;
   std::string err;
   std::string name;
   int flags = 0;
-  int tune[24] = {0};
+  int tune[kTuneKnobs] = {0};
 
   int64_t Mg = 0, row0 = 0, rows = 0, ncols_ext = 0;
   int64_t rows_pad = 0;
@@ -262,6 +264,11 @@
   int* d_osi = nullptr;
   int os_n = 0;
   int os_step_n = 0;
+  hipStream_t os_stream = nullptr;
+  hipEvent_t e_os_walk = nullptr, e_os_alpha = nullptr, e_os_ready = nullptr;
+  bool os_side_pending = false;
+  double* d_ospart = nullptr;
+  size_t ospart_cap = 0;
   const char* tap_what = nullptr;
   double* d_tap = nullptr;
   size_t tap_cap = 0, tap_count = 0;
@@ -365,7 +372,8 @@
   hipEvent_t a = nullptr, b = nullptr;
   bool on;
   bool marked = false;
-  Scope(lz_handle h_, int cls_, double bytes, double flops);
+  hipStream_t st;
+  Scope(lz_handle h_, int cls_, double bytes, double flops, hipStream_t stream = nullptr);
   ~Scope();
 };
 int drain_events(lz_handle h);
diff --git a/lanczos_amd/csrc/lz_internal.h b/lanczos_amd/csrc/lz_internal.h
--- a/lanczos_amd/csrc/lz_internal.h
+++ b/lanczos_amd/csrc/lz_internal.h
@@ -244,8 +244,8 @@
 int os_quad_sweep_blocks(int64_t len, bool wide8);
 void launch_os_quad_predict(const double* part, int np, double* nrm2, const double* chat, const double* G, const double* H, int n, int j,
                             const double* alpha, const double* beta, double* gout, int ldg, hipStream_t s);
-int launch_os_quad_sweep(double* V, int64_t ldv, int64_t len, int j, const double* g, int ldg, const double* z, const double* nrm2, double* part,
-                         bool wide8, hipStream_t s);
+int launch_os_quad_sweep(double* V, int64_t ldv, int64_t len, int j, const double* g, int ldg, const double* z, const double* bz, const double* nrm2,
+                         double* part, bool wide8, hipStream_t s);
 hipError_t launch_os_quad_post(const double* d, int ldp, const double* g, int ldg, double* G, double* H, int n, int j, const double* nrm2,
                                const double* alpha, double* beta, double tau, int* ist, double* elog, hipStream_t s);
 inline size_t omega_state_doubles(int n) { return (size_t)2 + (n + 2) + 3 * (size_t)(n + 1); }
@@ -261,6 +261,10 @@
 void launch_onereduce_finish(const double* buf, int ldp, double* alpha_last, double* beta_last, const double* uu_keep, hipStream_t s);
 int launch_three_term(double* r, const double* vj, const double* vjm1, const double* alpha, const double* beta,
                       int64_t len, double* part, hipStream_t s);
+int launch_three_term_z(int mode, double* out, const double* y, const double* zt, const double* xm, const double* alpha, const double* bt,
+                        const double* bm, int64_t len, double* part, hipStream_t s);
+void launch_final_sum_chain(const double* zpart, int nz, const double* apart, int na, double* beta_slot, double* alpha_slot, hipStream_t s);
+void launch_final_sum_root(const double* part, int np, double* out, const double* nrm2, double* root_out, hipStream_t s);
 void launch_gather(const double* x, const int32_t* idx, int64_t n, double* buf, hipStream_t s);
 
 void launch_bi(int first, int pend, int dots, double* x, double* y, const double* xs, const double* ys, const double* f,
diff --git a/lanczos_amd/csrc/lz_loops.hip b/lanczos_amd/csrc/lz_loops.hip
--- a/lanczos_amd/csrc/lz_loops.hip
+++ b/lanczos_amd/csrc/lz_loops.hip
@@ -394,8 +394,17 @@
 
 struct OneSweepState {
   double *G, *H, *chat, *g, *elog, *gq;
+  double* zp;
+  double* b3;
   int nb;
 };
+constexpr size_t kChainParts = 2048;
+static int one_sweep_join(lz_handle h) {
+  if (!h->os_side_pending) return LZ_OK;
+  h->os_side_pending = false;
+  LZ_HIP(h, hipStreamWaitEvent(h->stream, h->e_os_ready, 0));
+  return LZ_OK;
+}
 static void one_sweep_view(lz_handle h, int n, OneSweepState& st) {
   st.nb = os_sweep_blocks(h->rows_pad);
   st.G = h->d_os;
@@ -404,9 +413,23 @@
   st.g = st.chat + n + 1;
   st.elog = st.g + 2 * n + 2;
   st.gq = st.elog + n + 1;
+  st.zp = st.gq + (size_t)4 * (n + 4);
+  st.b3 = st.zp + kChainParts;
 }
 static int one_sweep_setup(lz_handle h, int n, OneSweepState& st, int pair_blocks = 0) {
-  const size_t os_doubles = (size_t)2 * n * n + (size_t)5 * n + 8 + (size_t)4 * (n + 4);
+  const size_t os_doubles = (size_t)2 * n * n + (size_t)5 * n + 8 + (size_t)4 * (n + 4) + kChainParts + 8;
+  LZ_TRY(one_sweep_join(h));
+  if (!h->os_stream) {
+    LZ_HIP(h, hipStreamCreateWithFlags(&h->os_stream, hipStreamNonBlocking));
+    LZ_HIP(h, hipEventCreateWithFlags(&h->e_os_walk, hipEventDisableTiming));
+    LZ_HIP(h, hipEventCreateWithFlags(&h->e_os_alpha, hipEventDisableTiming));
+    LZ_HIP(h, hipEventCreateWithFlags(&h->e_os_ready, hipEventDisableTiming));
+  }
+  const size_t ospart = (size_t)(h->rows / kTPB) + 64;
+  if (h->ospart_cap < ospart) {
+    LZ_TRY(dev_alloc(h, h->d_ospart, ospart));
+    h->ospart_cap = ospart;
+  }
   if (h->os_n < n) {
     LZ_TRY(dev_alloc(h, h->d_os, os_doubles));
     LZ_TRY(dev_alloc(h, h->d_osi, 8));
@@ -475,6 +498,7 @@
 }
 static int one_sweep_fused_iter(lz_handle h, int n, int j, const OneSweepState& st) {
   double* vj = basis_row(h, j);
+  LZ_TRY(one_sweep_join(h));
   LZ_TRY(one_sweep_step(h, n, j, st, j > 0));
   int npa = 0;
   if (j == 0) {
@@ -492,6 +516,7 @@
   return LZ_OK;
 }
 static int one_sweep_fused_tail(lz_handle h, int n) {
+  LZ_TRY(one_sweep_join(h));
   LZ_TRY(step_three_term(h, n - 1, n - 2, h->d_alpha + (n - 1), beta_slot(h, n, n - 1), true));
   h->r_state = 1;
   return LZ_OK;
@@ -518,6 +543,7 @@
   double* pp = st.g + n + 1;
   const int* scale = h->d_osi + 2;
   h->prof_iter = iter_sampled(h, j) || iter_sampled(h, j + 1);
+  LZ_TRY(one_sweep_join(h));
   LZ_TRY(step_three_term(h, j - 1, j - 2, h->d_alpha + (j - 1), h->d_beta + (j - 2), true));
   int npa = 0;
   LZ_TRY(step_scaling_spmv(h, n, j, h->d_r, h->d_r2, scale, &npa));
@@ -577,49 +603,108 @@
   const double M = (double)h->rows;
   const int ldg = n + 4;
   h->prof_iter = iter_sampled(h, j) || iter_sampled(h, j + 1) || iter_sampled(h, j + 2) || iter_sampled(h, j + 3);
-  LZ_TRY(step_three_term(h, j - 1, j - 2, h->d_alpha + (j - 1), h->d_beta + (j - 2), true));
-  double* src = h->d_r;
-  double* dst = h->d_r2;
+  const bool zchain = h->tune[15] != 12;
+  const bool side = zchain && h->tune[15] != 13;
+  if (!zchain) LZ_TRY(one_sweep_join(h));
+  const double* z = nullptr;
+  const double* zpart = nullptr;
   int npz = 0;
-  for (int t = 0; t < 3; ++t) {
-    int npa = 0;
-    LZ_TRY(step_scaling_spmv(h, n, j + t, src, dst, h->d_osi + 2, &npa));
-    LZ_TRY(step_final_sum(h, npa, h->d_alpha + (j + t), "final_sum(alpha)"));
-    LZ_TRY(step_three_term(h, j + t, j + t - 1, h->d_alpha + (j + t), h->d_beta + (j + t - 1), t < 2, &npz, dst));
-    std::swap(src, dst);
-  }
-  const double* z = src;
+  if (zchain) {
+    const double* b_open = h->os_side_pending ? st.b3 : h->d_beta + (j - 2);
+    auto three_term_z = [&](int mode, int t) {
+      Scope sc(h, LZ_K_THREE, 32.0 * M, (mode == 0 ? 6.0 : mode == 1 ? 8.0 : 9.0) * M);
+      npz = launch_three_term_z(mode, basis_row(h, j + t + 1), h->d_r, basis_row(h, j + t), basis_row(h, j + t - 1), h->d_alpha + (j + t),
+                                mode == 0 ? b_open : h->d_beta + (j + t - 1), mode == 2 ? h->d_beta + (j + t - 2) : nullptr, h->rows_pad, st.zp,
+                                h->stream);
+      return check_launch(h, mode == 0 ? "three_term(chain opening)" : "three_term(chain)");
+    };
+    LZ_TRY(three_term_z(0, -1));
+    for (int t = 0; t < 3; ++t) {
+      double* zt = basis_row(h, j + t);
+      int npa = 0;
+      {
+        Scope sc(h, LZ_K_SPMV, spmv_bytes(h, true), spmv_flops(h));
+        npa = launch_spmv_ell(h->csr, zt, h->d_r, zt, h->d_ospart, h->stream);
+        LZ_TRY(check_launch(h, "spmv(ell, chain)"));
+      }
+      {
+        Scope sc(h, LZ_K_FINAL, 0, 0);
+        launch_final_sum_chain(st.zp, npz, h->d_ospart, npa, h->d_beta + (j + t - 1), h->d_alpha + (j + t), h->stream);
+        LZ_TRY(check_launch(h, "final_sum(chain)"));
+      }
+      LZ_TRY(three_term_z(t == 0 ? 1 : 2, t));
+    }
+    z = basis_row(h, j + 3);
+    zpart = st.zp;
+  } else {
+    LZ_TRY(step_three_term(h, j - 1, j - 2, h->d_alpha + (j - 1), h->d_beta + (j - 2), true));
+    double* src = h->d_r;
+    double* dst = h->d_r2;
+    for (int t = 0; t < 3; ++t) {
+      int npa = 0;
+      LZ_TRY(step_scaling_spmv(h, n, j + t, src, dst, h->d_osi + 2, &npa));
+      LZ_TRY(step_final_sum(h, npa, h->d_alpha + (j + t), "final_sum(alpha)"));
+      LZ_TRY(step_three_term(h, j + t, j + t - 1, h->d_alpha + (j + t), h->d_beta + (j + t - 1), t < 2, &npz, dst));
+      std::swap(src, dst);
+    }
+    z = src;
+    zpart = h->d_part;
+  }
   const int ldp = os_quad_ldp(j);
+  LZ_TRY(one_sweep_join(h));
   {
     Scope sc(h, LZ_K_FINAL, 0, 0);
-    launch_os_quad_predict(h->d_part, npz, h->d_nrm2, st.chat, st.G, st.H, n, j, h->d_alpha + j, h->d_beta + (j - 1), st.gq, ldg, h->stream);
+    launch_os_quad_predict(zpart, npz, h->d_nrm2, st.chat, st.G, st.H, n, j, h->d_alpha + j, h->d_beta + (j - 1), st.gq, ldg, h->stream);
     LZ_TRY(check_launch(h, "one-sweep group predict"));
   }
   {
     Scope sc(h, LZ_K_UPDATE, 8.0 * j * M + 64.0 * M, 16.0 * (j + 1) * M);
-    launch_os_quad_sweep(h->d_V, h->ldv, h->rows_pad, j, st.gq, ldg, z, h->d_nrm2, h->d_part, wide8, h->stream);
+    launch_os_quad_sweep(h->d_V, h->ldv, h->rows_pad, j, st.gq, ldg, z, zchain ? h->d_beta + (j - 1) : nullptr, h->d_nrm2, h->d_part, wide8, h->stream);
     LZ_TRY(check_launch(h, "one-sweep group walk"));
   }
-  {
-    Scope sc(h, LZ_K_FINAL, 0, 0);
-    launch_final_rows_t(h->d_part, nbq, 4 * ldp, 3 * ldp + j + 4, h->d_c, h->stream);
+  hipStream_t ps = side ? h->os_stream : h->stream;
+  if (side) {
+    LZ_HIP(h, hipEventRecord(h->e_os_walk, h->stream));
+    LZ_HIP(h, hipStreamWaitEvent(h->os_stream, h->e_os_walk, 0));
+    h->os_side_pending = true;
+  }
+  {
+    Scope sc(h, LZ_K_FINAL, 0, 0, ps);
+    launch_final_rows_t(h->d_part, nbq, 4 * ldp, 3 * ldp + j + 4, h->d_c, ps);
     LZ_TRY(check_launch(h, "final_rows(one-sweep group)"));
     LZ_HIP(h, launch_os_quad_post(h->d_c, ldp, st.gq, ldg, st.G, st.H, n, j, h->d_nrm2, h->d_alpha + j, h->d_beta + (j - 1), kOneSweepTau, h->d_osi,
-                                  st.elog, h->stream));
+                                  st.elog, ps));
     LZ_TRY(check_launch(h, "one-sweep group post"));
   }
   {
     double* vj = basis_row(h, j + 3);
+    double* apart = zchain ? h->d_ospart : h->d_part;
     int npa = 0;
     {
       Scope sc(h, LZ_K_SPMV, spmv_bytes(h, true), spmv_flops(h));
-      npa = launch_spmv_ell(h->csr, vj, h->d_r, vj, h->d_part, h->stream);
+      npa = launch_spmv_ell(h->csr, vj, h->d_r, vj, apart, h->stream);
       LZ_TRY(check_launch(h, "spmv(ell)"));
     }
-    Scope sc(h, LZ_K_FINAL, 0, 0);
-    launch_os_sum_predict(h->d_part, npa, h->d_alpha + (j + 3), st.G, st.H, n, j + 3, h->d_alpha + (j + 3), h->d_beta + (j + 2), st.chat, true,
-                          j + 4 < n, h->stream);
-    LZ_TRY(check_launch(h, "final_sum(alpha) + one-sweep predict"));
+    if (side) {
+      {
+        Scope sc(h, LZ_K_FINAL, 0, 0);
+        launch_final_sum_root(apart, npa, h->d_alpha + (j + 3), h->d_nrm2, st.b3, h->stream);
+        LZ_TRY(check_launch(h, "final_sum(alpha, b3)"));
+      }
+      LZ_HIP(h, hipEventRecord(h->e_os_alpha, h->stream));
+      LZ_HIP(h, hipStreamWaitEvent(h->os_stream, h->e_os_alpha, 0));
+      if (j + 4 < n) {
+        Scope sc(h, LZ_K_FINAL, 0, 0, ps);
+        launch_os_sum_predict(nullptr, 0, h->d_alpha + (j + 3), st.G, st.H, n, j + 3, h->d_alpha + (j + 3), h->d_beta + (j + 2), st.chat, true, true, ps);
+        LZ_TRY(check_launch(h, "one-sweep predict(side)"));
+      }
+      LZ_HIP(h, hipEventRecord(h->e_os_ready, h->os_stream));
+    } else {
+      Scope sc(h, LZ_K_FINAL, 0, 0);
+      launch_os_sum_predict(apart, npa, h->d_alpha + (j + 3), st.G, st.H, n, j + 3, h->d_alpha + (j + 3), h->d_beta + (j + 2), st.chat, true,
+                            j + 4 < n, h->stream);
+      LZ_TRY(check_launch(h, "final_sum(alpha) + one-sweep predict"));
+    }
   }
   h->last_os_quads += 1;
   return LZ_OK;
@@ -716,6 +801,7 @@
   h->last_os_pairs = pairs;
   h->last_os_quads = quads;
   LZ_TRY(rc);
+  LZ_TRY(one_sweep_join(h));
   LZ_HIP(h, hipStreamSynchronize(h->stream));
   if (blocks) *blocks = nb;
   return LZ_OK;
@@ -726,6 +812,7 @@
   if (h->os_step_n != n || !h->d_os) return fail(h, LZ_ERR_STATE, "one-sweep step: no state set for this basis (lz_os_state_set after lz_basis_alloc)");
   OneSweepState st;
   one_sweep_view(h, n, st);
+  LZ_TRY(one_sweep_join(h));
   auto get = [&](void* dst, const void* src, size_t bytes) {
     return dst ? hipMemcpyAsync(dst, src, bytes, hipMemcpyDeviceToHost, h->stream) : hipSuccess;
   };
@@ -749,6 +836,7 @@
 }
 
 int one_sweep_raw_get(lz_handle h, int j0, int count, double* rows, double* part, int64_t part_count) {
+  LZ_TRY(one_sweep_join(h));
   if (rows) {
     if (count < 1 || j0 < 0 || j0 + count > h->n) return fail(h, LZ_ERR_ARG, "lz_os_raw_get: rows out of range");
     LZ_HIP(h, hipMemcpy2DAsync(rows, (size_t)h->rows_pad * sizeof(double), h->d_V + (int64_t)j0 * h->ldv, (size_t)h->ldv * sizeof(double),
@@ -795,7 +883,7 @@
   const bool knob_auto = h->tune[15] == 0;
 #endif
   const bool one_sweep_ok = one_rank && full_fused && default_kernels && !(f & LZ_FLAG_OVERLAP_HALO) && n >= 2 && n <= kOneSweepMaxN;
-  if (h->tune[15] >= 6 && h->tune[15] <= 11 && one_sweep_ok) return LOOP_ONE_SWEEP;
+  if (h->tune[15] >= 6 && h->tune[15] <= 13 && one_sweep_ok) return LOOP_ONE_SWEEP;
   if (!knob_auto || !full_fused || !default_kernels) return LOOP_SIX;
   if (one_rank && qp.G <= 8 && n <= 4096 && h->part_cap >= fused_coff(h) + (size_t)(n + 16) * (size_t)qp.G) return LOOP_FUSED_SMALL;
   if (!(f & LZ_FLAG_OVERLAP_HALO) && h->rows_pad <= kThreeTermFusedMaxRows) return LOOP_THREE_TERM_FUSED;
diff --git a/lanczos_amd/csrc/lz_reorth.hip b/lanczos_amd/csrc/lz_reorth.hip
--- a/lanczos_amd/csrc/lz_reorth.hip
+++ b/lanczos_amd/csrc/lz_reorth.hip
@@ -1124,6 +1124,93 @@
   if (g < 1) g = 1;
   hipLaunchKernelGGL(k_three_term, dim3((int)g), dim3(kTPB), 0, s, r, vj, vjm1, alpha, beta, n2, part);
   return (int)g;
+}
+
+template <int MODE>
+__global__ __launch_bounds__(kTPB) void k_three_term_z(double* __restrict__ out, const double* __restrict__ y, const double* __restrict__ zt,
+                                                      const double* __restrict__ xm, const double* __restrict__ alpha,
+                                                      const double* __restrict__ bt, const double* __restrict__ bm, int64_t n2,
+                                                      double* __restrict__ part) {
+  __shared__ double sm[kTPB / 64];
+  const double a = alpha[0];
+  const double b = bt[0];
+  const double bp = MODE == 2 ? bm[0] : 1.0;
+  double2* o2 = reinterpret_cast<double2*>(out);
+  const double2* y2 = reinterpret_cast<const double2*>(y);
+  const double2* v2 = reinterpret_cast<const double2*>(zt);
+  const double2* m2 = reinterpret_cast<const double2*>(xm);
+  double acc = 0.0;
+  for (int64_t i = (int64_t)blockIdx.x * kTPB + threadIdx.x; i < n2; i += (int64_t)gridDim.x * kTPB) {
+    double2 x = y2[i];
+    double2 v, m;
+    if (MODE == 0) {
+      v = ld_stream<1>(v2 + i);
+      m = ld_stream<1>(m2 + i);
+    } else {
+      v = v2[i];
+      m = m2[i];
+      x.x = x.x / b;
+      x.y = x.y / b;
+      v.x = v.x / b;
+      v.y = v.y / b;
+    }
+    if (MODE == 2) {
+      m.x = m.x / bp;
+      m.y = m.y / bp;
+    }
+    x.x = x.x - v.x * a;
+    x.y = x.y - v.y * a;
+    x.x = x.x - m.x * b;
+    x.y = x.y - m.y * b;
+    o2[i] = x;
+    acc = fma(x.x, x.x, acc);
+    acc = fma(x.y, x.y, acc);
+  }
+  acc = block_sum(acc, sm);
+  if (threadIdx.x == 0) part[blockIdx.x] = acc;
+}
+
+int launch_three_term_z(int mode, double* out, const double* y, const double* zt, const double* xm, const double* alpha, const double* bt,
+                        const double* bm, int64_t len, double* part, hipStream_t s) {
+  const int64_t n2 = len >> 1;
+  int64_t g = (n2 + kTPB - 1) / kTPB;
+  if (g > 2048) g = 2048;
+  if (g < 1) g = 1;
+#define LZ_TTZ_GO(MM) hipLaunchKernelGGL(k_three_term_z<MM>, dim3((int)g), dim3(kTPB), 0, s, out, y, zt, xm, alpha, bt, bm, n2, part)
+  switch (mode) {
+    case 0: LZ_TTZ_GO(0); break;
+    case 1: LZ_TTZ_GO(1); break;
+    default: LZ_TTZ_GO(2); break;
+  }
+#undef LZ_TTZ_GO
+  return (int)g;
+}
+
+__global__ __launch_bounds__(kFinalThreads) void k_final_sum_chain(const double* __restrict__ zpart, int nz, const double* __restrict__ apart,
+                                                                  int na, double* __restrict__ beta_slot, double* __restrict__ alpha_slot) {
+  __shared__ double sm[2][kFinalThreads / 64];
+  const double zz = final_sum_1024(zpart, nz, sm[0]);
+  const double za = final_sum_1024(apart, na, sm[1]);
+  if (threadIdx.x == 0) {
+    beta_slot[0] = sqrt(zz);
+    alpha_slot[0] = za / zz;
+  }
+}
+void launch_final_sum_chain(const double* zpart, int nz, const double* apart, int na, double* beta_slot, double* alpha_slot, hipStream_t s) {
+  hipLaunchKernelGGL(k_final_sum_chain, dim3(1), dim3(kFinalThreads), 0, s, zpart, nz, apart, na, beta_slot, alpha_slot);
+}
+
+__global__ __launch_bounds__(kFinalThreads) void k_final_sum_root(const double* __restrict__ part, int np, double* __restrict__ out,
+                                                                 const double* __restrict__ nrm2, double* __restrict__ root_out) {
+  __shared__ double sm[kFinalThreads / 64];
+  const double t = final_sum_1024(part, np, sm);
+  if (threadIdx.x == 0) {
+    out[0] = t;
+    root_out[0] = sqrt(nrm2[0]);
+  }
+}
+void launch_final_sum_root(const double* part, int np, double* out, const double* nrm2, double* root_out, hipStream_t s) {
+  hipLaunchKernelGGL(k_final_sum_root, dim3(1), dim3(kFinalThreads), 0, s, part, np, out, nrm2, root_out);
 }
 
 __global__ __launch_bounds__(kTPB) void k_three_term_self(double* __restrict__ r, const double* __restrict__ u, const double* __restrict__ vm,
@@ -1522,10 +1609,14 @@
                                                                  double* __restrict__ chat, int predict) {
   __shared__ double sm[kFinalThreads / 64];
   __shared__ double s_sum;
-  const double t = final_sum_1024(part, np, sm);
-  if (threadIdx.x == 0) {
-    sum_out[0] = t;
-    s_sum = t;
+  if (predict == 2) {
+    if (threadIdx.x == 0) s_sum = alpha_j[0];
+  } else {
+    const double t = final_sum_1024(part, np, sm);
+    if (threadIdx.x == 0) {
+      sum_out[0] = t;
+      s_sum = t;
+    }
   }
   if (!predict) return;
   __syncthreads();
@@ -1546,7 +1637,9 @@
 
 void launch_os_sum_predict(const double* part, int np, double* sum_out, const double* G, double* H, int n, int j, const double* alpha_j,
                            const double* beta_j, double* chat, bool fused, bool predict, hipStream_t s) {
-  if (fused)
+  if (fused && !part)
+    hipLaunchKernelGGL(k_os_sum_predict<true>, dim3(1), dim3(kFinalThreads), 0, s, part, 0, sum_out, G, H, n, j, alpha_j, beta_j, chat, 2);
+  else if (fused)
     hipLaunchKernelGGL(k_os_sum_predict<true>, dim3(1), dim3(kFinalThreads), 0, s, part, np, sum_out, G, H, n, j, alpha_j, beta_j, chat, predict ? 1 : 0);
   else
     hipLaunchKernelGGL(k_os_sum_predict<false>, dim3(1), dim3(kFinalThreads), 0, s, part, np, sum_out, G, H, n, j, alpha_j, beta_j, chat, predict ? 1 : 0);
@@ -1978,8 +2071,8 @@
 
 template <int P, int RU>
 __global__ __launch_bounds__(kTPB) void k_os_quad_sweep(double* __restrict__ V, int64_t ldv, int n2, int j, const double* __restrict__ g, int ldg,
-                                                       const double* __restrict__ zbuf, const double* __restrict__ nrm2, int ldp,
-                                                       double* __restrict__ part) {
+                                                       const double* __restrict__ zbuf, const double* __restrict__ bz,
+                                                       const double* __restrict__ nrm2, int ldp, double* __restrict__ part) {
   extern __shared__ double keep[];
   constexpr int NV = 4 * RU;
   const int lane = threadIdx.x & 63, wv = threadIdx.x >> 6;
@@ -1998,11 +2091,19 @@
   double2 x[4][P];
   double sx[4][P], sy[4][P];
   {
-    const double2* z2 = reinterpret_cast<const double2*>(zbuf);
+    const double2* z2 = bz ? V2 + (int64_t)(j + 3) * ld2 : reinterpret_cast<const double2*>(zbuf);
+    double bt[3] = {1.0, 1.0, 1.0};
+    if (bz) {
+#pragma unroll
+      for (int t = 0; t < 3; ++t) bt[t] = bz[t];
+    }
 #pragma unroll
     for (int p = 0; p < P; ++p) {
 #pragma unroll
-      for (int t = 0; t < 3; ++t) x[t][p] = V2[(int64_t)(j + t) * ld2 + pos[p]];
+      for (int t = 0; t < 3; ++t) {
+        x[t][p] = V2[(int64_t)(j + t) * ld2 + pos[p]];
+        if (bz) x[t][p] = make_double2(x[t][p].x / bt[t], x[t][p].y / bt[t]);
+      }
       const double2 zz = z2[pos[p]];
       x[3][p] = make_double2(zz.x / b3, zz.y / b3);
 #pragma unroll
@@ -2116,15 +2217,15 @@
 }
 int os_quad_ldp(int j) { return qtw_ldp(j + 4); }
 
-int launch_os_quad_sweep(double* V, int64_t ldv, int64_t len, int j, const double* g, int ldg, const double* z, const double* nrm2, double* part,
-                         bool wide8, hipStream_t s) {
+int launch_os_quad_sweep(double* V, int64_t ldv, int64_t len, int j, const double* g, int ldg, const double* z, const double* bz, const double* nrm2,
+                         double* part, bool wide8, hipStream_t s) {
   const int64_t n2 = len >> 1;
   const int P = os_quad_sweep_p(n2, wide8);
   const int grid = (int)((n2 + (int64_t)kTPB * P - 1) / ((int64_t)kTPB * P));
   const int ldp = os_quad_ldp(j);
   const size_t lds = os_quad_lds_bytes(ldp);
 #define LZ_OSQ_GO(PP, RR) \
-  hipLaunchKernelGGL((k_os_quad_sweep<PP, RR>), dim3(grid), dim3(kTPB), lds, s, V, ldv, (int)n2, j, g, ldg, z, nrm2, ldp, part)
+  hipLaunchKernelGGL((k_os_quad_sweep<PP, RR>), dim3(grid), dim3(kTPB), lds, s, V, ldv, (int)n2, j, g, ldg, z, bz, nrm2, ldp, part)
   switch (P) {
     case 8: LZ_OSQ_GO(8, 1); break;
     case 4: LZ_OSQ_GO(4, 2); break;
```

Result: faster. 2022 (median of 6 runs) (+5.0%).
